# violetdenim/c3dgs

Hardware: AMD Instinct MI355X
Metric: raster views/sec fwd+bwd @1920x1080 (higher is better)
Workload: dtype f32; 1 GPU; BASELINE.json configs[2]: synth-v1 3M Gaussians, SH deg 3, indexed-camera rasterizer (QAT inner loop), mark_visible+fwd+bwd, 1 view/step/GPU; gaussians=3000000, width=1920, height=1080, sh_codebook=304096, gaussian_codebook=754096, parallelism=replicas x1

## Files before the change

c3dgs_amd/csrc/binning.hip:

```cpp
#include "common.hpp"
#include <rocprim/device/device_radix_sort.hpp>
#include <rocprim/iterator/counting_iterator.hpp>

namespace c3dgs {

size_t scan_temp_bytes(int P)
{
    size_t a = 0, b = 0;
    (void)rocprim::radix_sort_pairs(nullptr, b, (const uint32_t*)nullptr, (uint32_t*)nullptr, (const uint32_t*)nullptr,
                                    (uint32_t*)nullptr, (size_t)P, 0u, 32u);
    size_t m = a > b ? a : b;
    const size_t os = onesweep_depth_temp_bytes(P);
    if (os > m) m = os;
    return m < 256 ? 256 : m;
}

size_t sort_temp_bytes(int R, int end_bit, int key_bytes)
{
    size_t bytes = 0;
    if (key_bytes == 4)
        (void)rocprim::radix_sort_pairs(nullptr, bytes, (const uint32_t*)nullptr, (uint32_t*)nullptr,
                                        (const uint32_t*)nullptr, (uint32_t*)nullptr, (size_t)R, 0u, (unsigned)end_bit);
    else
        (void)rocprim::radix_sort_pairs(nullptr, bytes, (const uint16_t*)nullptr, (uint16_t*)nullptr,
                                        (const uint32_t*)nullptr, (uint32_t*)nullptr, (size_t)R, 0u, (unsigned)end_bit);
    const size_t os = onesweep_tile_temp_bytes(R, end_bit, key_bytes);
    if (os > bytes) bytes = os;
    const size_t reuse = align_up((size_t)(R > 0 ? R : 1));
    if (reuse > bytes) bytes = reuse;
    return bytes < 256 ? 256 : bytes;
}

__global__ void __launch_bounds__(256)
gather_u64_kernel(int n, const uint32_t* __restrict__ idx, const uint2* __restrict__ src, uint2* __restrict__ dst)
{
    const int i = blockIdx.x * 256 + threadIdx.x;
    if (i < n) dst[i] = src[idx[i]];
}

size_t depth_sort_clear_bytes(int P)
{
    return (onesweep_enabled() && (size_t)P < ((size_t)1 << 30)) ? onesweep_depth_clear_bytes(P) : 0;
}
size_t tile_sort_clear_bytes(int R, int end_bit, int key_bytes)
{
    return (onesweep_enabled() && (size_t)R < ((size_t)1 << 30)) ? onesweep_tile_clear_bytes(R, end_bit, key_bytes) : 0;
}

hipError_t run_depth_sort(void* temp, size_t temp_bytes, const uint32_t* kin, uint32_t* kout, const uint32_t* vin,
                          uint32_t* vout, int P, const uint2* rects, uint2* rects_sorted, hipStream_t s, bool ctrl_cleared,
                          bool rects_fit_bytes)
{
    if (onesweep_enabled() && (size_t)P < ((size_t)1 << 30))
        return onesweep_depth_sort(temp, temp_bytes, kin, kout, vin, vout, P, rects, rects_sorted, s, ctrl_cleared, rects_fit_bytes);
    hipError_t e = vin ? rocprim::radix_sort_pairs(temp, temp_bytes, kin, kout, vin, vout, (size_t)P, 0u, 32u, s)
                       : rocprim::radix_sort_pairs(temp, temp_bytes, kin, kout, rocprim::counting_iterator<uint32_t>(0u), vout,
                                                   (size_t)P, 0u, 32u, s);
    if (e != hipSuccess) return e;
    gather_u64_kernel<<<(P + 255) / 256, 256, 0, s>>>(P, vout, rects, rects_sorted);
    return hipGetLastError();
}

hipError_t run_tile_sort(void* temp, size_t temp_bytes, const void* kin, void* kout, int key_bytes, const uint32_t* vin,
                         uint32_t* vout, int R, int end_bit, hipStream_t s, bool ctrl_cleared)
{
    if (key_bytes == 4) {
        if (onesweep_enabled() && (size_t)R < ((size_t)1 << 30))
            return onesweep_tile_sort32(temp, temp_bytes, (const uint32_t*)kin, (uint32_t*)kout, vin, vout, R, end_bit, s, ctrl_cleared);
        return rocprim::radix_sort_pairs(temp, temp_bytes, (const uint32_t*)kin, (uint32_t*)kout, vin, vout, (size_t)R, 0u, (unsigned)end_bit, s);
    }
    if (onesweep_enabled() && (size_t)R < ((size_t)1 << 30))
        return onesweep_tile_sort(temp, temp_bytes, (const uint16_t*)kin, (uint16_t*)kout, vin, vout, R, end_bit, s, ctrl_cleared);
    return rocprim::radix_sort_pairs(temp, temp_bytes, (const uint16_t*)kin, (uint16_t*)kout, vin, vout, (size_t)R, 0u, (unsigned)end_bit, s);
}

}
```

c3dgs_amd/csrc/c_abi.hip:

```cpp
#include "common.hpp"
#include <cstdlib>
#include <cstring>
#include <mutex>
#include <vector>

namespace c3dgs {

static thread_local std::string g_last_error;
void set_error(const std::string& msg) { g_last_error = msg; }

enum Stage { ST_MARK_VISIBLE, ST_PREPROCESS, ST_DEPTH_SORT, ST_SCAN, ST_DUPLICATE, ST_SORT, ST_RANGES, ST_RENDER_FWD, ST_ZERO_PARTIALS,
             ST_RENDER_BWD, ST_BWD_PREPROCESS, ST_WDIST, ST_VQ_ACC, ST_VQ_APPLY, ST_LOSS_FWD, ST_LOSS_BWD,
             ST_QAT_OBSERVE, ST_QAT_CODEBOOKS, ST_QAT_VISIBLE, ST_QAT_POINTS, ST_QAT_POINTS_BWD, ST_QAT_CODEBOOKS_BWD, ST_ADAM, ST_COUNT };
static const char* kStageNames[ST_COUNT] = { "mark_visible", "preprocess", "depth_sort", "scan", "duplicate_with_keys", "sort",
                                             "identify_ranges", "render_forward", "zero_partials", "render_backward",
                                             "backward_preprocess", "weighted_distance", "vq_accumulate", "vq_apply", "l1_ssim_forward",
                                             "l1_ssim_backward", "qat_observe", "qat_codebooks", "qat_visible", "qat_points",
                                             "qat_points_backward", "qat_codebooks_backward", "adam_step" };
struct ProfRec { int stage; hipEvent_t a, b; };
static std::mutex g_prof_mu;
static bool g_prof_on = false;
static int g_prof_only = -1;
static std::vector<ProfRec> g_prof_recs;
static std::vector<hipEvent_t> g_prof_pool;

struct StageTimer {
    bool on; int stage; hipStream_t s; hipEvent_t a{}, b{};
    StageTimer(int stage_, hipStream_t s_) : on(g_prof_on && (g_prof_only < 0 || g_prof_only == stage_)), stage(stage_), s(s_)
    {
        if (!on) return;
        std::lock_guard<std::mutex> lk(g_prof_mu);
        auto get = [&](hipEvent_t& e) {
            if (!g_prof_pool.empty()) { e = g_prof_pool.back(); g_prof_pool.pop_back(); }
            else if (hipEventCreate(&e) != hipSuccess) on = false;
        };
        get(a); get(b);
        if (on) (void)hipEventRecord(a, s);
    }
    ~StageTimer()
    {
        if (!on) return;
        (void)hipEventRecord(b, s);
        std::lock_guard<std::mutex> lk(g_prof_mu);
        g_prof_recs.push_back({ stage, a, b });
    }
};

struct HostRead {
    uint32_t* pinned = nullptr;
    uint32_t* dev = nullptr;
    uint32_t seq = 0;
    hipEvent_t ev{};
    HostRead()
    {
        const char* e = std::getenv("C3DGS_HOST_READ_COPY");
        const bool want_map = !(e && e[0] == '1');
        if (want_map && hipHostMalloc((void**)&pinned, 64, hipHostMallocMapped | hipHostMallocPortable | hipHostMallocCoherent) == hipSuccess) {
            void* d = nullptr;
            if (hipHostGetDevicePointer(&d, pinned, 0) == hipSuccess) dev = (uint32_t*)d;
            std::memset(pinned, 0, 64);
        } else {
            (void)hipGetLastError();
            if (hipHostMalloc((void**)&pinned, 64, hipHostMallocDefault) != hipSuccess) { pinned = nullptr; return; }
        }
        if (hipEventCreateWithFlags(&ev, hipEventDisableTiming) != hipSuccess) { (void)hipHostFree(pinned); pinned = nullptr; dev = nullptr; }
    }
};
static HostRead& host_read()
{
    static thread_local HostRead h;
    return h;
}

static int validate(const c3dgs_raster_params* p, bool indexed, bool is_backward)
{
    if (!p) return fail(C3DGS_E_INVALID, "params is NULL");
    if (p->P < 0 || p->W <= 0 || p->H <= 0) return fail(C3DGS_E_INVALID, "P, W, H must be non-negative / positive");
    if (p->P == 0) return C3DGS_OK;
    if (!p->means3D) return fail(C3DGS_E_INVALID, "means3D must have dimensions (num_points, 3)");
    if (!p->background || !p->viewmatrix || !p->projmatrix || !p->campos)
        return fail(C3DGS_E_INVALID, "background, viewmatrix, projmatrix and campos are required");
    if (!is_backward && !p->opacities)
        return fail(C3DGS_E_INVALID, "opacities is required");
    if ((p->sh == nullptr) == (p->colors_precomp == nullptr))
        return fail(C3DGS_E_INVALID, "Please provide excatly one of either SHs or precomputed colors!");
    const bool has_sr = p->scales != nullptr && p->rotations != nullptr;
    if ((p->scales != nullptr) != (p->rotations != nullptr) || has_sr == (p->cov3D_precomp != nullptr))
        return fail(C3DGS_E_INVALID, "Please provide exactly one of either scale/rotation pair or precomputed 3D covariance!");
    if (p->sh) {
        if (p->D < 0 || p->D > 3) return fail(C3DGS_E_INVALID, "SH degree must be in [0,3]");
        if (p->M < (p->D + 1) * (p->D + 1)) return fail(C3DGS_E_INVALID, "sh has fewer coefficients than the active degree needs");
    }
    if (indexed) {
        if (p->sh && !p->sh_indices) return fail(C3DGS_E_INVALID, "indexed rasterizer: sh_indices is required with sh");
        if (has_sr && (!p->g_indices || !p->scale_factors))
            return fail(C3DGS_E_INVALID, "indexed rasterizer: g_indices and scale_factors are required with scales/rotations");
    } else if (p->sh_indices || p->g_indices || p->scale_factors) {
        return fail(C3DGS_E_INVALID, "non-indexed rasterizer: sh_indices / g_indices / scale_factors must be NULL");
    }
    if (tiles_x(p->W) > 65535 || tiles_y(p->H) > 65535) return fail(C3DGS_E_INVALID, "image too large for 16-bit tile coordinates");
    if ((unsigned long long)tiles_x(p->W) * tiles_x(p->W) * tiles_y(p->H) >= (1ull << 32))
        return fail(C3DGS_E_INVALID, "image too large: (tiles per row)^2 x (tile rows) must stay below 2^32");
    return C3DGS_OK;
}

static int forward_impl(const c3dgs_raster_params* pp, bool indexed, c3dgs_resize_fn geom_resize, void* geom_user,
                        c3dgs_resize_fn binning_resize, void* binning_user, c3dgs_resize_fn image_resize, void* image_user,
                        float* out_color, int32_t* radii, int32_t* num_rendered, void* stream_)
{
    if (int rc = validate(pp, indexed, false)) return rc;
    if (!out_color || !num_rendered) return fail(C3DGS_E_INVALID, "out_color and num_rendered are required");
    if (!geom_resize || !binning_resize || !image_resize) return fail(C3DGS_E_INVALID, "resize callbacks are required");
    c3dgs_raster_params p = *pp;
    if (!indexed) { p.sh_indices = nullptr; p.g_indices = nullptr; p.scale_factors = nullptr; }
    hipStream_t s = (hipStream_t)stream_;
    const int P = p.P, W = p.W, H = p.H;
    const int gx = tiles_x(W), gy = tiles_y(H), T = gx * gy;
    *num_rendered = 0;

    c3dgs_image_layout IL; image_layout(W, H, &IL);
    void* img_base = image_resize(image_user, IL.total_bytes);
    if (!img_base) return fail(C3DGS_E_ALLOC, "image buffer allocation failed");
    const ImgPtrs img = img_ptrs(img_base, W, H);

    if (P == 0) {
        C3DGS_HIP_TRY(hipMemsetAsync(out_color, 0, (size_t)3 * W * H * sizeof(float), s));
        C3DGS_HIP_TRY(hipMemsetAsync(img_base, 0, IL.total_bytes, s));
        return C3DGS_OK;
    }
    if (!radii) return fail(C3DGS_E_INVALID, "radii is required");

    c3dgs_geom_layout GL; geom_layout(P, &GL);
    void* geom_base = geom_resize(geom_user, GL.total_bytes + geom_gtab_bytes(p));
    if (!geom_base) return fail(C3DGS_E_ALLOC, "geometry buffer allocation failed");
    const GeomPtrs g = geom_ptrs(geom_base, P);

    uint32_t* sort_err = onesweep_error_word();
    if (!sort_err) return fail(C3DGS_E_HIP, "cannot resolve the sort error word");
    HostRead& hr = host_read();
    if (!hr.pinned) return fail(C3DGS_E_HIP, "pinned host buffer allocation failed");
    const uint32_t seq = hr.dev ? ++hr.seq : 0u;
    if (hr.dev && seq == 0u) hr.seq = 1u;
    const uint32_t want_seq = hr.dev ? hr.seq : 0u;
    const size_t dclear = depth_sort_clear_bytes(P) <= g.scan_temp_bytes ? depth_sort_clear_bytes(P) : 0;
    { StageTimer t_(ST_PREPROCESS, s);
      if (geom_gtab_bytes(p)) launch_pack_codebook(p, g.gtab, s);
      launch_preprocess(p, g, radii, img.ranges, sort_err, g.scan_temp, dclear / 16, hr.dev, want_seq, s); }
    C3DGS_STAGE("preprocess", p.debug, s);
    if (!hr.dev) {
        C3DGS_HIP_TRY(hipMemcpyAsync(hr.pinned, g.block_base + (P + 255) / 256, 2 * sizeof(uint32_t), hipMemcpyDeviceToHost, s));
        C3DGS_HIP_TRY(hipEventRecord(hr.ev, s));
    }
    { StageTimer t_(ST_DEPTH_SORT, s);
      C3DGS_HIP_TRY(run_depth_sort(g.scan_temp, g.scan_temp_bytes, g.depth_keys, g.depth_keys_sorted, nullptr, g.depth_order, P,
                                   reinterpret_cast<const uint2*>(g.rects), g.sorted_offsets, s, dclear != 0,
                                   gx <= 255 && gy <= 255)); }
    C3DGS_STAGE("depth_sort", p.debug, s);
    if (p.debug && onesweep_timed_out(s)) return fail(C3DGS_E_HIP, "depth sort: look-back timed out");
    { StageTimer t_(ST_SCAN, s); launch_depth_order_scan(P, g, s); }
    C3DGS_STAGE("scan", p.debug, s);
    if (hr.dev) {
        volatile uint32_t* pad = hr.pinned;
        bool seen = false;
        for (long spins = 0; !seen; spins++) {
            seen = __atomic_load_n(&pad[2], __ATOMIC_ACQUIRE) == want_seq;
            if (!seen && (spins & 0xffff) == 0xffff) {
                const hipError_t q = hipStreamQuery(s);
                if (q == hipErrorNotReady) continue;
                if (q != hipSuccess) return fail(C3DGS_E_HIP, std::string("num_rendered read: ") + hipGetErrorString(q));
                seen = __atomic_load_n(&pad[2], __ATOMIC_ACQUIRE) == want_seq;
                if (!seen) {
                    C3DGS_HIP_TRY(hipMemcpyAsync(hr.pinned, g.block_base + (P + 255) / 256, 2 * sizeof(uint32_t), hipMemcpyDeviceToHost, s));
                    C3DGS_HIP_TRY(hipStreamSynchronize(s));
                    seen = true;
                }
            }
        }
    } else {
        hipError_t q = hipErrorNotReady;
        for (long spins = 0; spins < 20000000L && (q = hipEventQuery(hr.ev)) == hipErrorNotReady; spins++) { }
        if (q == hipErrorNotReady) q = hipEventSynchronize(hr.ev);
        if (q != hipSuccess) return fail(C3DGS_E_HIP, std::string("num_rendered read: ") + hipGetErrorString(q));
    }
    const uint32_t R_u = hr.pinned[0];
    if (hr.pinned[1] != 0) {
        C3DGS_HIP_TRY(hipMemsetAsync(sort_err, 0, sizeof(uint32_t), s));
        return fail(C3DGS_E_HIP, "radix sort look-back timed out in an earlier rasterizer call on this device: that call's "
                                 "image is NaN and its gradients are invalid (flag cleared, this call was not run)");
    }
    if (R_u > 0x7fffffffu) return fail(C3DGS_E_INVALID, "num_rendered overflows int32");
    const int R = (int)R_u;
    *num_rendered = R;

    c3dgs_binning_layout BL; binning_layout(R, W, H, &BL);
    void* bin_base = binning_resize(binning_user, BL.total_bytes);
    if (!bin_base) return fail(C3DGS_E_ALLOC, "binning buffer allocation failed");
    const BinPtrs b = bin_ptrs(bin_base, R, W, H);

    if (R > 0) {
        const int end_bit = (int)higher_msb((uint32_t)T);
        size_t tclear = tile_sort_clear_bytes(R, end_bit, b.key_bytes);
        if (tclear > b.sort_temp_bytes) tclear = 0;
        { StageTimer t_(ST_DUPLICATE, s); launch_duplicate_with_keys(P, g, b, gx, sort_err, b.sort_temp, tclear / 16, s); }
        C3DGS_STAGE("duplicate_with_keys", p.debug, s);
        { StageTimer t_(ST_SORT, s);
          C3DGS_HIP_TRY(run_tile_sort(b.sort_temp, b.sort_temp_bytes, b.keys_unsorted, b.keys_sorted, b.key_bytes, b.values_unsorted,
                                      b.point_list, R, end_bit, s, tclear != 0)); }
        C3DGS_STAGE("sort", p.debug, s);
        if (p.debug && onesweep_timed_out(s)) return fail(C3DGS_E_HIP, "tile sort: look-back timed out");
        { StageTimer t_(ST_RANGES, s); launch_identify_ranges(R, b.keys_sorted, b.key_bytes, img.ranges, sort_err, s); }
        C3DGS_STAGE("identify_ranges", p.debug, s);
    }
    { StageTimer t_(ST_RENDER_FWD, s);
      launch_render_forward(W, H, img, b.point_list, g.splat, p.background, out_color, (uint8_t*)b.sort_temp, sort_err, s); }
    C3DGS_STAGE("render_forward", p.debug, s);
    return C3DGS_OK;
}

static int backward_impl(const c3dgs_raster_params* pp, bool indexed, const int32_t* radii, const void* geom_buffer,
                         const void* binning_buffer, const void* image_buffer, int32_t R, const float* dL_dout_color,
                         c3dgs_resize_fn ws_resize, void* ws_user, const c3dgs_raster_grads* grads, void* stream_)
{
    if (int rc = validate(pp, indexed, true)) return rc;
    if (!grads) return fail(C3DGS_E_INVALID, "grads is NULL");
    c3dgs_raster_params p = *pp;
    if (!indexed) { p.sh_indices = nullptr; p.g_indices = nullptr; p.scale_factors = nullptr; }
    hipStream_t s = (hipStream_t)stream_;
    const int P = p.P, W = p.W, H = p.H;

    void* cb_zero = nullptr;
    size_t cb_zero16 = 0;
    if (indexed) {
        const size_t n_sh = (grads->dL_dsh && p.sh) ? (size_t)p.SHS * p.M * 3 * sizeof(float) : 0;
        const size_t n_rot = (grads->dL_drotations && p.scales) ? (size_t)p.GS * 4 * sizeof(float) : 0;
        const size_t n_sc = (grads->dL_dscales && p.scales) ? (size_t)p.GS * 3 * sizeof(float) : 0;
        char* a_sh = (char*)grads->dL_dsh; char* a_rot = (char*)grads->dL_drotations; char* a_sc = (char*)grads->dL_dscales;
        if (n_sh && n_rot && n_sc && a_rot == a_sh + n_sh && a_sc == a_rot + n_rot) {
            const size_t n = n_sh + n_rot + n_sc;
            if (p.P > 0 && R >= 0 && ((uintptr_t)a_sh & 15u) == 0) {
                cb_zero = a_sh; cb_zero16 = n / 16;
                if (n % 16) C3DGS_HIP_TRY(hipMemsetAsync(a_sh + cb_zero16 * 16, 0, n % 16, s));
            } else {
                C3DGS_HIP_TRY(hipMemsetAsync(a_sh, 0, n, s));
            }
        } else {
            if (n_sh) C3DGS_HIP_TRY(hipMemsetAsync(a_sh, 0, n_sh, s));
            if (n_sc) C3DGS_HIP_TRY(hipMemsetAsync(a_sc, 0, n_sc, s));
            if (n_rot) C3DGS_HIP_TRY(hipMemsetAsync(a_rot, 0, n_rot, s));
        }
    }
    if (P == 0) return C3DGS_OK;
    if (!radii || !geom_buffer || !image_buffer || !dL_dout_color || (R > 0 && !binning_buffer))
        return fail(C3DGS_E_INVALID, "radii, forward buffers and dL_dout_color are required");
    if (!ws_resize) return fail(C3DGS_E_INVALID, "workspace callback is required");
    if (R < 0) return fail(C3DGS_E_INVALID, "R must be >= 0");

    const GeomPtrs g = geom_ptrs(const_cast<void*>(geom_buffer), P);
    const ImgPtrs img = img_ptrs(const_cast<void*>(image_buffer), W, H);
    const size_t ws_bytes = c3dgs_backward_workspace_bytes(P, R);
    float* partials = (float*)ws_resize(ws_user, ws_bytes);
    if (!partials) return fail(C3DGS_E_ALLOC, "backward workspace allocation failed");

    const size_t r1 = (size_t)(R > 0 ? R : 1), p256 = ((size_t)P + 1023) / 1024 * 1024;
    uint8_t* touched = (uint8_t*)partials + align_up(r1 * PARTIAL_FLOATS * sizeof(float));
    uint32_t* tile_order = img.tile_order;
    uint32_t* live_ids = (uint32_t*)(touched + align_up(r1)) + 65536;
    uint32_t* live_slots = live_ids + p256;
    uint32_t* live_count = live_slots + p256;
    { StageTimer t_(ST_ZERO_PARTIALS, s);
      launch_backward_prep(R > 0 ? W : 0, H, img, tile_order, touched, align_up(r1) / 16, R > 0 ? nullptr : cb_zero,
                           R > 0 ? 0 : cb_zero16, s); }
    if (R > 0) {
        const BinPtrs b = bin_ptrs(const_cast<void*>(binning_buffer), R, W, H);
        { StageTimer t_(ST_RENDER_BWD, s);
          launch_render_backward(W, H, img, b.point_list, g.splat, g.block_base, p.background, dL_dout_color, partials, touched,
                                 (const uint8_t*)b.sort_temp, tile_order, cb_zero, cb_zero16, s); }
        C3DGS_STAGE("render_backward", p.debug, s);
    }
    { StageTimer t_(ST_BWD_PREPROCESS, s);
      launch_backward_preprocess(p, radii, g, partials, touched, live_count, live_ids, live_slots, *grads, s); }
    C3DGS_STAGE("backward_preprocess", p.debug, s);
    return C3DGS_OK;
}

}

using namespace c3dgs;

extern "C" {

const char* c3dgs_last_error(void) { return g_last_error.c_str(); }

int c3dgs_profile_enable(int on)
{
    std::lock_guard<std::mutex> lk(g_prof_mu);
    g_prof_on = on != 0;
    return C3DGS_OK;
}

int c3dgs_profile_only(const char* stage_name)
{
    std::lock_guard<std::mutex> lk(g_prof_mu);
    g_prof_only = -1;
    if (!stage_name || !*stage_name) return C3DGS_OK;
    for (int i = 0; i < ST_COUNT; i++)
        if (std::strcmp(stage_name, kStageNames[i]) == 0) { g_prof_only = i; return C3DGS_OK; }
    return fail(C3DGS_E_INVALID, std::string("profile_only: unknown stage ") + stage_name);
}

int c3dgs_profile_read(c3dgs_stage_time* out, int capacity)
{
    std::vector<ProfRec> recs;
    {
        std::lock_guard<std::mutex> lk(g_prof_mu);
        recs.swap(g_prof_recs);
    }
    double total[ST_COUNT] = { 0 };
    long long count[ST_COUNT] = { 0 };
    for (auto& r : recs) {
        float ms = 0.f;
        if (hipEventSynchronize(r.b) == hipSuccess && hipEventElapsedTime(&ms, r.a, r.b) == hipSuccess) {
            total[r.stage] += (double)ms;
            count[r.stage]++;
        }
    }
    {
        std::lock_guard<std::mutex> lk(g_prof_mu);
        for (auto& r : recs) { g_prof_pool.push_back(r.a); g_prof_pool.push_back(r.b); }
    }
    int n = 0;
    for (int i = 0; i < ST_COUNT && n < capacity; i++) {
        if (!count[i]) continue;
        std::memset(&out[n], 0, sizeof(out[n]));
        std::strncpy(out[n].name, kStageNames[i], sizeof(out[n].name) - 1);
        out[n].total_ms = total[i];
        out[n].count = count[i];
        n++;
    }
    return n;
}
int c3dgs_abi_version(void) { return C3DGS_ABI_VERSION; }

int c3dgs_debug_sort_times(uint64_t* out )
{
    unsigned long long v[512];
    if (!out || os_read_times(v)) return fail(C3DGS_E_INVALID, "debug_sort_times: not a C3DGS_OS_TIMING build");
    for (int i = 0; i < 512; i++) out[i] = (uint64_t)v[i];
    return C3DGS_OK;
}

int c3dgs_debug_gather_probe(int32_t kind, int64_t n, void* table, const uint32_t* index, uint32_t* out, void* stream)
{
    if (n < 0 || !table || !out || (kind != 0 && !index)) return fail(C3DGS_E_INVALID, "debug_gather_probe: bad arguments");
    if (launch_gather_probe(kind, (size_t)n, table, index, out, (hipStream_t)stream)) return fail(C3DGS_E_INVALID, "debug_gather_probe: kind must be 0..3");
    return C3DGS_OK;
}

int c3dgs_debug_lane_counters(uint64_t* out, void* stream)
{
    if (!out) return fail(C3DGS_E_INVALID, "debug_lane_counters: NULL buffer");
    unsigned long long v[16];
    if (read_lane_counters(v, (hipStream_t)stream)) return fail(C3DGS_E_HIP, "debug_lane_counters: copy failed");
    for (int i = 0; i < 16; i++) out[i] = (uint64_t)v[i];
    return C3DGS_OK;
}

size_t c3dgs_debug_sort_temp_bytes(int32_t key_bytes, int64_t n, int32_t end_bit)
{
    if (n <= 0 || n > 0x3fffffff) return 256;
    return key_bytes == 2 ? onesweep_tile_temp_bytes((int)n, end_bit) : onesweep_depth_temp_bytes((int)n);
}

int c3dgs_debug_sort_pairs(int32_t key_bytes, int64_t n, int32_t end_bit, const void* keys_in, void* keys_out,
                           const uint32_t* values_in, uint32_t* values_out, void* temp, size_t temp_bytes, void* stream)
{
    if ((key_bytes != 2 && key_bytes != 4) || n < 0 || n > 0x3fffffff || end_bit < 1 || end_bit > 8 * key_bytes)
        return fail(C3DGS_E_INVALID, "debug_sort_pairs: bad arguments");
    if (key_bytes == 4 && end_bit != 32) return fail(C3DGS_E_INVALID, "debug_sort_pairs: 4-byte keys are sorted on all 32 bits");
    if (n == 0) return C3DGS_OK;
    if (!keys_in || !keys_out || !values_in || !values_out || !temp) return fail(C3DGS_E_INVALID, "debug_sort_pairs: NULL buffer");
    hipStream_t s = (hipStream_t)stream;
    if (key_bytes == 2)
        C3DGS_HIP_TRY(onesweep_tile_sort(temp, temp_bytes, (const uint16_t*)keys_in, (uint16_t*)keys_out, values_in, values_out, (int)n,
                                         end_bit, s));
    else
        C3DGS_HIP_TRY(onesweep_depth_sort(temp, temp_bytes, (const uint32_t*)keys_in, (uint32_t*)keys_out, values_in, values_out, (int)n,
                                          nullptr, nullptr, s));
    C3DGS_STAGE("debug_sort_pairs", 1, s);
    if (onesweep_timed_out(s)) return fail(C3DGS_E_HIP, "debug_sort_pairs: look-back timed out");
    return C3DGS_OK;
}

int c3dgs_get_geom_layout(int32_t P, c3dgs_geom_layout* out)
{
    if (!out || P < 0) return fail(C3DGS_E_INVALID, "bad arguments");
    geom_layout(P, out);
    return C3DGS_OK;
}
int c3dgs_get_binning_layout(int32_t R, int32_t W, int32_t H, c3dgs_binning_layout* out)
{
    if (!out || R < 0 || W <= 0 || H <= 0) return fail(C3DGS_E_INVALID, "bad arguments");
    binning_layout(R, W, H, out);
    return C3DGS_OK;
}
int c3dgs_get_image_layout(int32_t W, int32_t H, c3dgs_image_layout* out)
{
    if (!out || W <= 0 || H <= 0) return fail(C3DGS_E_INVALID, "bad arguments");
    image_layout(W, H, out);
    return C3DGS_OK;
}
size_t c3dgs_backward_workspace_bytes(int32_t P, int32_t R)
{
    const size_t r = (size_t)(R > 0 ? R : 1), p256 = ((size_t)(P > 0 ? P : 1) + 1023) / 1024 * 1024;
    return align_up(r * PARTIAL_FLOATS * sizeof(float)) + align_up(r) + 65536 * sizeof(uint32_t) +
           (2 * p256 + p256 / 256) * sizeof(uint32_t) + 256;
}

int c3dgs_mark_visible(int32_t P, const float* means3D, const float* viewmatrix, const float* projmatrix, uint8_t* present,
                       void* stream)
{
    (void)projmatrix;
    if (P < 0) return fail(C3DGS_E_INVALID, "P must be >= 0");
    if (P == 0) return C3DGS_OK;
    if (!means3D || !viewmatrix || !present) return fail(C3DGS_E_INVALID, "means3D, viewmatrix and present are required");
    { StageTimer t_(ST_MARK_VISIBLE, (hipStream_t)stream); launch_mark_visible(P, means3D, viewmatrix, present, (hipStream_t)stream); }
    C3DGS_STAGE("mark_visible", 0, (hipStream_t)stream);
    return C3DGS_OK;
}

int c3dgs_mark_visible_pose(int32_t P, const float* means3D, const float* extrinsic_vector, uint8_t* present, void* stream)
{
    if (P < 0) return fail(C3DGS_E_INVALID, "P must be >= 0");
    if (P == 0) return C3DGS_OK;
    if (!means3D || !extrinsic_vector || !present) return fail(C3DGS_E_INVALID, "means3D, extrinsic_vector and present are required");
    { StageTimer t_(ST_MARK_VISIBLE, (hipStream_t)stream); launch_mark_visible_pose(P, means3D, extrinsic_vector, present, (hipStream_t)stream); }
    C3DGS_STAGE("mark_visible", 0, (hipStream_t)stream);
    return C3DGS_OK;
}

int c3dgs_camera_from_pose(const float* extrinsic_vector, float inv_tan_half_fovx, float inv_tan_half_fovy, float* viewmatrix,
                           float* projmatrix, float* campos, void* stream)
{
    if (!extrinsic_vector || !viewmatrix || !projmatrix || !campos) return fail(C3DGS_E_INVALID, "camera_from_pose: NULL pointer");
    launch_camera_from_pose(extrinsic_vector, inv_tan_half_fovx, inv_tan_half_fovy, viewmatrix, projmatrix, campos, (hipStream_t)stream);
    C3DGS_STAGE("camera_from_pose", 0, (hipStream_t)stream);
    return C3DGS_OK;
}

int c3dgs_rasterize_gaussians(const c3dgs_raster_params* p, c3dgs_resize_fn geom_resize, void* geom_user,
                              c3dgs_resize_fn binning_resize, void* binning_user, c3dgs_resize_fn image_resize,
                              void* image_user, float* out_color, int32_t* radii, int32_t* num_rendered, void* stream)
{
    return forward_impl(p, false, geom_resize, geom_user, binning_resize, binning_user, image_resize, image_user, out_color,
                        radii, num_rendered, stream);
}

int c3dgs_rasterize_gaussians_indexed(const c3dgs_raster_params* p, c3dgs_resize_fn geom_resize, void* geom_user,
                                      c3dgs_resize_fn binning_resize, void* binning_user, c3dgs_resize_fn image_resize,
                                      void* image_user, float* out_color, int32_t* radii, int32_t* num_rendered, void* stream)
{
    return forward_impl(p, true, geom_resize, geom_user, binning_resize, binning_user, image_resize, image_user, out_color,
                        radii, num_rendered, stream);
}

int c3dgs_rasterize_gaussians_backward(const c3dgs_raster_params* p, const int32_t* radii, const void* geom_buffer,
                                       const void* binning_buffer, const void* image_buffer, int32_t R,
                                       const float* dL_dout_color, c3dgs_resize_fn workspace_resize, void* workspace_user,
                                       const c3dgs_raster_grads* grads, void* stream)
{
    return backward_impl(p, false, radii, geom_buffer, binning_buffer, image_buffer, R, dL_dout_color, workspace_resize,
                         workspace_user, grads, stream);
}

int c3dgs_rasterize_gaussians_backward_indexed(const c3dgs_raster_params* p, const int32_t* radii, const void* geom_buffer,
                                               const void* binning_buffer, const void* image_buffer, int32_t R,
                                               const float* dL_dout_color, c3dgs_resize_fn workspace_resize,
                                               void* workspace_user, const c3dgs_raster_grads* grads, void* stream)
{
    return backward_impl(p, true, radii, geom_buffer, binning_buffer, image_buffer, R, dL_dout_color, workspace_resize,
                         workspace_user, grads, stream);
}

int c3dgs_weighted_distance(int64_t N, int32_t C, int32_t K, const float* coefs, const int64_t* gather,
                            const float* codebook, float* out_dist, int64_t* out_idx, void* stream)
{
    if (N < 0 || C < 0 || K <= 0) return fail(C3DGS_E_INVALID, "coefs and codebook must have same number of channels");
    if (N == 0) return C3DGS_OK;
    if (!coefs || !codebook || !out_dist || !out_idx) return fail(C3DGS_E_INVALID, "ceofs and codebook must have dimension 2");
    {
        StageTimer t_(ST_WDIST, (hipStream_t)stream);
        if (launch_weighted_distance(N, C, K, coefs, gather, codebook, out_dist, out_idx, (hipStream_t)stream))
            return fail(C3DGS_E_INVALID, "unsupported channel count");
    }
    C3DGS_STAGE("weighted_distance", 0, (hipStream_t)stream);
    return C3DGS_OK;
}

size_t c3dgs_weighted_distance_ws_bytes(int64_t N, int32_t C, int32_t K) { return wd_ws_bytes(N, C, K); }

int c3dgs_weighted_distance_ws(int64_t N, int32_t C, int32_t K, const float* coefs, const int64_t* gather, const float* codebook,
                               float* out_dist, int64_t* out_idx, void* ws, size_t ws_bytes, void* stream)
{
    if (N < 0 || C < 0 || K <= 0) return fail(C3DGS_E_INVALID, "coefs and codebook must have same number of channels");
    if (N == 0) return C3DGS_OK;
    if (!coefs || !codebook || !out_dist || !out_idx) return fail(C3DGS_E_INVALID, "ceofs and codebook must have dimension 2");
    {
        StageTimer t_(ST_WDIST, (hipStream_t)stream);
        if (launch_weighted_distance(N, C, K, coefs, gather, codebook, out_dist, out_idx, (hipStream_t)stream, ws, ws ? ws_bytes : 0))
            return fail(C3DGS_E_INVALID, "unsupported channel count");
    }
    C3DGS_STAGE("weighted_distance", 0, (hipStream_t)stream);
    return C3DGS_OK;
}

int c3dgs_vq_accumulate(int64_t B, int32_t K, int32_t D, const float* x, const float* w, const int64_t* gather,
                        const int64_t* idx, const float* dist, float* S, double* dist_sum, void* stream)
{
    if (B < 0 || K <= 0 || D <= 0) return fail(C3DGS_E_INVALID, "bad sizes");
    if (B == 0) return C3DGS_OK;
    if (!x || !w || !idx || !S) return fail(C3DGS_E_INVALID, "x, w, idx and S are required");
    { StageTimer t_(ST_VQ_ACC, (hipStream_t)stream); launch_vq_accumulate(B, K, D, x, w, gather, idx, dist, S, dist_sum, (hipStream_t)stream); }
    C3DGS_STAGE("vq_accumulate", 0, (hipStream_t)stream);
    return C3DGS_OK;
}

int c3dgs_vq_sums(int64_t B, int32_t K, int32_t D, const float* x, const float* w, const int64_t* gather,
                  const float* codebook, float* dist, int64_t* idx, float* S, double* dist_sum, void* ws, size_t ws_bytes,
                  void* stream)
{
    if (B < 0 || K <= 0 || D <= 0) return fail(C3DGS_E_INVALID, "bad sizes");
    if (!S || !dist_sum) return fail(C3DGS_E_INVALID, "S and dist_sum are required");
    C3DGS_HIP_TRY(hipMemsetAsync(S, 0, (size_t)K * (D + 1) * sizeof(float), (hipStream_t)stream));
    C3DGS_HIP_TRY(hipMemsetAsync(dist_sum, 0, sizeof(double), (hipStream_t)stream));
    if (B == 0) return C3DGS_OK;
    if (!x || !w || !codebook || !dist || !idx) return fail(C3DGS_E_INVALID, "x, w, codebook, dist and idx are required");
    {
        StageTimer t_(ST_WDIST, (hipStream_t)stream);
        if (launch_weighted_distance(B, K, D, x, gather, codebook, dist, idx, (hipStream_t)stream, ws, ws ? ws_bytes : 0))
            return fail(C3DGS_E_INVALID, "unsupported channel count");
    }
    C3DGS_STAGE("weighted_distance", 0, (hipStream_t)stream);
    return c3dgs_vq_accumulate(B, K, D, x, w, gather, idx, dist, S, dist_sum, stream);
}

int c3dgs_vq_step_supported(int32_t K, int32_t D, const float* x, const float* codebook, const void* ws, size_t ws_bytes)
{
    return (K > 0 && D > 0 && wd_presplit_supported(K, D, x, codebook, ws, ws_bytes)) ? 1 : 0;
}

int c3dgs_vq_step_sums(int32_t step, int64_t B, int32_t K, int32_t D, const float* x, const float* w, const int64_t* gather,
                       const float* codebook, float* dist, int64_t* idx, float* S, double* dist_sum, void* ws, size_t ws_bytes,
                       void* stream)
{
    hipStream_t s = (hipStream_t)stream;
    if (step < 0 || B <= 0 || K <= 0 || D <= 0) return fail(C3DGS_E_INVALID, "vq_step_sums: bad sizes");
    if (!x || !w || !codebook || !dist || !idx || !S || !dist_sum) return fail(C3DGS_E_INVALID, "vq_step_sums: NULL argument");
    if (!wd_presplit_supported(K, D, x, codebook, ws, ws_bytes))
        return fail(C3DGS_E_INVALID, "vq_step_sums: shape / scratch not served by the fused step (see c3dgs_vq_step_supported)");
    if (step == 0) {
        C3DGS_HIP_TRY(hipMemsetAsync(S, 0, (size_t)K * (D + 1) * sizeof(float), s));
        C3DGS_HIP_TRY(hipMemsetAsync(dist_sum, 0, sizeof(double), s));
    }
    {
        StageTimer t_(ST_WDIST, s);
        if (launch_weighted_distance(B, K, D, x, gather, codebook, dist, idx, s, ws, ws_bytes, step == 0 ? -1 : (step & 1)))
            return fail(C3DGS_E_INVALID, "vq_step_sums: unsupported shape");
        if (step == 0) launch_vq_seed_words(K, D, ws, s);
    }
    C3DGS_STAGE("weighted_distance", 0, s);
    { StageTimer t_(ST_VQ_ACC, s);
      launch_vq_accumulate(B, K, D, x, w, gather, idx, dist, S, dist_sum, s, vq_next_absmax_word(K, D, ws, step & 1)); }
    C3DGS_STAGE("vq_accumulate", 0, s);
    return C3DGS_OK;
}

int c3dgs_vq_step_apply(int32_t step, int32_t K, int32_t D, float* S, float* codebook, float* entry_importance, float decay,
                        float alpha, float eps, int32_t scale_normalize, void* ws, size_t ws_bytes, void* stream)
{
    if (step < 0 || K <= 0 || D <= 0 || !S || !codebook || !entry_importance) return fail(C3DGS_E_INVALID, "vq_step_apply: bad arguments");
    { StageTimer t_(ST_VQ_APPLY, (hipStream_t)stream);
      if (launch_vq_apply_split(K, D, S, codebook, entry_importance, decay, alpha, eps, scale_normalize, ws, ws_bytes, step & 1, (hipStream_t)stream))
          return fail(C3DGS_E_INVALID, "vq_step_apply: shape / scratch not served by the fused step (see c3dgs_vq_step_supported)"); }
    C3DGS_STAGE("vq_apply", 0, (hipStream_t)stream);
    return C3DGS_OK;
}

int c3dgs_debug_wd_scores(int64_t N, int32_t C, int32_t K, const float* coefs, const float* codebook, float* scores, void* ws,
                          size_t ws_bytes, float* out_dist, int64_t* out_idx, void* stream)
{
    if (!coefs || !codebook || !scores || !out_dist || !out_idx) return fail(C3DGS_E_INVALID, "debug_wd_scores: bad arguments");
    if (launch_wd_debug_scores(N, C, K, coefs, codebook, scores, ws, ws_bytes, out_dist, out_idx, (hipStream_t)stream))
        return fail(C3DGS_E_INVALID, "debug_wd_scores: K = 48, 1 <= N <= 256, C >= 32 and scratch of c3dgs_weighted_distance_ws_bytes");
    return C3DGS_OK;
}

int c3dgs_vq_apply(int32_t K, int32_t D, const float* S, float* codebook, float* entry_importance, float decay,
                   float alpha, float eps, int32_t scale_normalize, void* stream)
{
    if (K <= 0 || D <= 0 || !S || !codebook || !entry_importance) return fail(C3DGS_E_INVALID, "bad arguments");
    { StageTimer t_(ST_VQ_APPLY, (hipStream_t)stream); launch_vq_apply(K, D, S, codebook, entry_importance, decay, alpha, eps, scale_normalize, (hipStream_t)stream); }
    C3DGS_STAGE("vq_apply", 0, (hipStream_t)stream);
    return C3DGS_OK;
}

size_t c3dgs_morton_workspace_bytes(int32_t P) { return morton_workspace_bytes(P); }

int c3dgs_morton_order(int32_t P, const float* xyz, int64_t* codes, int64_t* order, void* workspace, void* stream)
{
    if (P < 0) return fail(C3DGS_E_INVALID, "P must be >= 0");
    if (P == 0) return C3DGS_OK;
    if (!xyz || !codes || !order || !workspace) return fail(C3DGS_E_INVALID, "morton_order: bad arguments");
    if (run_morton_order(P, xyz, codes, order, workspace, (hipStream_t)stream)) return fail(C3DGS_E_HIP, "morton_order failed");
    C3DGS_STAGE("morton_order", 0, (hipStream_t)stream);
    return C3DGS_OK;
}

int c3dgs_abs_accumulate(int64_t n, const float* g, float* acc, void* stream)
{
    if (n < 0 || (n > 0 && (!g || !acc))) return fail(C3DGS_E_INVALID, "abs_accumulate: bad arguments");
    launch_abs_accumulate(n, g, acc, (hipStream_t)stream);
    C3DGS_STAGE("abs_accumulate", 0, (hipStream_t)stream);
    return C3DGS_OK;
}

int c3dgs_adam_step(int32_t n_tensors, const c3dgs_adam_tensor* tensors, double beta1, double beta2, double eps, void* stream)
{
    if (n_tensors < 0 || n_tensors > C3DGS_ADAM_MAX_TENSORS) return fail(C3DGS_E_INVALID, "adam_step: between 0 and 16 tensors per call");
    if (n_tensors == 0) return C3DGS_OK;
    if (!tensors) return fail(C3DGS_E_INVALID, "adam_step: tensors is NULL");
    for (int k = 0; k < n_tensors; k++)
        if (tensors[k].n > 0 && (!tensors[k].param || !tensors[k].grad || !tensors[k].exp_avg || !tensors[k].exp_avg_sq))
            return fail(C3DGS_E_INVALID, "adam_step: NULL tensor pointer");
    { StageTimer t_(ST_ADAM, (hipStream_t)stream); launch_adam(n_tensors, tensors, beta1, beta2, eps, (hipStream_t)stream); }
    C3DGS_STAGE("adam_step", 0, (hipStream_t)stream);
    return C3DGS_OK;
}

int c3dgs_extract_rot_scale(int32_t n, const float* cov6, float* rot, float* scale, void* stream)
{
    if (n < 0) return fail(C3DGS_E_INVALID, "extract_rot_scale: n must be >= 0");
    if (n == 0) return C3DGS_OK;
    if (!cov6 || !rot || !scale || (reinterpret_cast<uintptr_t>(rot) & 15)) return fail(C3DGS_E_INVALID, "extract_rot_scale: bad arguments");
    launch_extract_rot_scale(n, cov6, rot, scale, (hipStream_t)stream);
    C3DGS_STAGE("extract_rot_scale", 0, (hipStream_t)stream);
    return C3DGS_OK;
}

int c3dgs_l1_ssim_forward(int32_t C, int32_t H, int32_t W, const float* img, const float* gt, float* dmaps, double* sums,
                          void* stream)
{
    if (C <= 0 || H <= 0 || W <= 0 || !img || !gt || !sums) return fail(C3DGS_E_INVALID, "l1_ssim_forward: bad arguments");
    hipStream_t s = (hipStream_t)stream;
    C3DGS_HIP_TRY(hipMemsetAsync(sums, 0, 128 * sizeof(double), s));
    const size_t n = (size_t)C * H * W;
    {
        StageTimer t_(ST_LOSS_FWD, s);
        launch_l1_ssim_forward(C, H, W, img, gt, dmaps, dmaps ? dmaps + n : nullptr, dmaps ? dmaps + 2 * n : nullptr, sums, s);
    }
    C3DGS_STAGE("l1_ssim_forward", 0, s);
    return C3DGS_OK;
}

int c3dgs_l1_ssim_value(const double* sums, double l1_scale, double ssim_scale, double constant, float* out, void* stream)
{
    if (!sums || !out) return fail(C3DGS_E_INVALID, "l1_ssim_value: bad arguments");
    launch_l1_ssim_value(sums, l1_scale, ssim_scale, constant, out, (hipStream_t)stream);
    C3DGS_STAGE("l1_ssim_value", 0, (hipStream_t)stream);
    return C3DGS_OK;
}

int c3dgs_l1_ssim_backward(int32_t C, int32_t H, int32_t W, const float* img, const float* gt, const float* dmaps,
                           const float* grad_loss, float l1_coeff, float ssim_coeff, float* dL_dimg, void* stream)
{
    if (C <= 0 || H <= 0 || W <= 0 || !img || !gt || !dmaps || !grad_loss || !dL_dimg)
        return fail(C3DGS_E_INVALID, "l1_ssim_backward: bad arguments");
    hipStream_t s = (hipStream_t)stream;
    const size_t n = (size_t)C * H * W;
    {
        StageTimer t_(ST_LOSS_BWD, s);
        launch_l1_ssim_backward(C, H, W, img, gt, dmaps, dmaps + n, dmaps + 2 * n, grad_loss, l1_coeff, ssim_coeff, dL_dimg, s);
    }
    C3DGS_STAGE("l1_ssim_backward", 0, s);
    return C3DGS_OK;
}

size_t c3dgs_image_metrics_ws_bytes(int32_t N, int32_t C, int32_t H, int32_t W) { return image_metrics_ws_bytes(N, C, H, W); }

int c3dgs_image_metrics(int32_t N, int32_t C, int32_t H, int32_t W, const float* img, const float* gt, void* ws, size_t ws_bytes,
                        double* out, void* stream)
{
    if (N <= 0 || C <= 0 || H <= 0 || W <= 0) return fail(C3DGS_E_INVALID, "image_metrics: N, C, H and W must be positive");
    if (image_metrics_workgroups(N, C, H, W) > IMAGE_METRICS_MAX_WORKGROUPS)
        return fail(C3DGS_E_INVALID, "image_metrics: size overflow (N * C * H * W too large for one call; split the batch)");
    if (!img || !gt || !ws || !out) return fail(C3DGS_E_INVALID, "image_metrics: img, gt, ws and out are required");
    if (reinterpret_cast<uintptr_t>(ws) & 7) return fail(C3DGS_E_INVALID, "image_metrics: ws must be 8-byte aligned");
    const size_t need = image_metrics_ws_bytes(N, C, H, W);
    if (ws_bytes < need)
        return fail(C3DGS_E_INVALID, "image_metrics: ws too small (" + std::to_string(ws_bytes) + " bytes, need " +
                                         std::to_string(need) + ")");
    launch_image_metrics(N, C, H, W, img, gt, (double*)ws, out, (hipStream_t)stream);
    C3DGS_STAGE("image_metrics", 0, (hipStream_t)stream);
    return C3DGS_OK;
}

static int qat_validate(const c3dgs_qat_params* q, const char* who)
{
    if (!q) return fail(C3DGS_E_INVALID, std::string(who) + ": params is NULL");
    if (q->P < 0 || q->GS < 0 || q->SHS < 0 || q->M < 1) return fail(C3DGS_E_INVALID, std::string(who) + ": bad sizes");
    if (!q->state) return fail(C3DGS_E_INVALID, std::string(who) + ": state is required");
    if (q->features_dc && q->M > 1 && !q->features_rest)
        return fail(C3DGS_E_INVALID, std::string(who) + ": features_rest is required with features_dc when M > 1");
    if (reinterpret_cast<uintptr_t>(q->rotation) & 15) return fail(C3DGS_E_INVALID, std::string(who) + ": rotation must be 16-byte aligned");
    return C3DGS_OK;
}
static bool misaligned16(const void* p) { return (reinterpret_cast<uintptr_t>(p) & 15) != 0; }

size_t c3dgs_qat_workspace_bytes(void) { return qat_workspace_bytes(); }
size_t c3dgs_qat_scan_bytes(int32_t P) { return qat_scan_bytes(P); }

int c3dgs_qat_observe(const c3dgs_qat_params* q, void* workspace, void* stream)
{
    if (int rc = qat_validate(q, "qat_observe")) return rc;
    if (!workspace) return fail(C3DGS_E_INVALID, "qat_observe: workspace is required");
    { StageTimer t_(ST_QAT_OBSERVE, (hipStream_t)stream); launch_qat_observe(*q, workspace, (hipStream_t)stream); }
    C3DGS_STAGE("qat_observe", 0, (hipStream_t)stream);
    return C3DGS_OK;
}

int c3dgs_qat_codebooks(const c3dgs_qat_params* q, float* scales_n, float* rotations, float* shs, void* stream)
{
    if (int rc = qat_validate(q, "qat_codebooks")) return rc;
    if (misaligned16(rotations) || misaligned16(shs)) return fail(C3DGS_E_INVALID, "qat_codebooks: outputs must be 16-byte aligned");
    { StageTimer t_(ST_QAT_CODEBOOKS, (hipStream_t)stream); launch_qat_codebooks(*q, scales_n, rotations, shs, (hipStream_t)stream); }
    C3DGS_STAGE("qat_codebooks", 0, (hipStream_t)stream);
    return C3DGS_OK;
}

int c3dgs_qat_codebooks_backward(const c3dgs_qat_params* q, const float* dL_dscales_n, const float* dL_drotations,
                                 const float* dL_dshs, float* dL_dscaling, float* dL_drotation, float* dL_dfeatures_dc,
                                 float* dL_dfeatures_rest, void* stream)
{
    if (int rc = qat_validate(q, "qat_codebooks_backward")) return rc;
    if (misaligned16(dL_drotations) || misaligned16(dL_drotation) || misaligned16(dL_dshs))
        return fail(C3DGS_E_INVALID, "qat_codebooks_backward: rotation / sh gradients must be 16-byte aligned");
    if (dL_dshs && q->features_dc && (!dL_dfeatures_dc || (q->M > 1 && !dL_dfeatures_rest)))
        return fail(C3DGS_E_INVALID, "qat_codebooks_backward: dL_dfeatures_dc / dL_dfeatures_rest are required with dL_dshs");
    {
        StageTimer t_(ST_QAT_CODEBOOKS_BWD, (hipStream_t)stream);
        launch_qat_codebooks_backward(*q, dL_dscales_n, dL_drotations, dL_dshs, dL_dscaling, dL_drotation, dL_dfeatures_dc,
                                      dL_dfeatures_rest, (hipStream_t)stream);
    }
    C3DGS_STAGE("qat_codebooks_backward", 0, (hipStream_t)stream);
    return C3DGS_OK;
}

int c3dgs_qat_visible(const c3dgs_qat_params* q, const float* viewmatrix, uint8_t* visible, int32_t* rank, int32_t* count,
                      void* scan_workspace, void* stream)
{
    if (int rc = qat_validate(q, "qat_visible")) return rc;
    if (!count) return fail(C3DGS_E_INVALID, "qat_visible: count is required");
    hipStream_t s = (hipStream_t)stream;
    if (q->P == 0) { C3DGS_HIP_TRY(hipMemsetAsync(count, 0, sizeof(int32_t), s)); return C3DGS_OK; }
    if (!q->xyz || !viewmatrix || !visible || !rank || !scan_workspace) return fail(C3DGS_E_INVALID, "qat_visible: bad arguments");
    { StageTimer t_(ST_QAT_VISIBLE, s); C3DGS_HIP_TRY(run_qat_visible(*q, viewmatrix, visible, rank, count, scan_workspace, s)); }
    C3DGS_STAGE("qat_visible", 0, s);
    return C3DGS_OK;
}

int c3dgs_qat_points(const c3dgs_qat_params* q, const uint8_t* visible, const int32_t* rank, const int64_t* sh_indices,
                     const int64_t* g_indices, float* means3D, float* opacities, float* scale_factors, int64_t* sh_indices_out,
                     int64_t* g_indices_out, void* stream)
{
    if (int rc = qat_validate(q, "qat_points")) return rc;
    if ((visible == nullptr) != (rank == nullptr)) return fail(C3DGS_E_INVALID, "qat_points: visible and rank go together");
    {
        StageTimer t_(ST_QAT_POINTS, (hipStream_t)stream);
        launch_qat_points(*q, visible, rank, sh_indices, g_indices, means3D, opacities, scale_factors, sh_indices_out,
                          g_indices_out, (hipStream_t)stream);
    }
    C3DGS_STAGE("qat_points", 0, (hipStream_t)stream);
    return C3DGS_OK;
}

int c3dgs_qat_points_backward(const c3dgs_qat_params* q, const uint8_t* visible, const int32_t* rank, const float* dL_dmeans3D,
                              const float* dL_dmeans2D, const float* dL_dopacities, const float* dL_dscale_factors,
                              float* dL_dxyz, float* dL_dscreenspace, float* dL_dopacity, float* dL_dscaling_factor, void* stream)
{
    if (int rc = qat_validate(q, "qat_points_backward")) return rc;
    if ((visible == nullptr) != (rank == nullptr)) return fail(C3DGS_E_INVALID, "qat_points_backward: visible and rank go together");
    if ((dL_dopacity && dL_dopacities && !q->opacity) || (dL_dscaling_factor && dL_dscale_factors && !q->scaling_factor))
        return fail(C3DGS_E_INVALID, "qat_points_backward: the raw opacity / scaling_factor are needed to recompute the masks");
    {
        StageTimer t_(ST_QAT_POINTS_BWD, (hipStream_t)stream);
        launch_qat_points_backward(*q, visible, rank, dL_dmeans3D, dL_dmeans2D, dL_dopacities, dL_dscale_factors, dL_dxyz,
                                   dL_dscreenspace, dL_dopacity, dL_dscaling_factor, (hipStream_t)stream);
    }
    C3DGS_STAGE("qat_points_backward", 0, (hipStream_t)stream);
    return C3DGS_OK;
}

int c3dgs_qat_quantize(const c3dgs_qat_params* q, int32_t scaling_is_exp, int8_t* opacity, int8_t* scaling, int8_t* scaling_factor,
                       int8_t* rotation, int8_t* features_dc, int8_t* features_rest, void* stream)
{
    if (int rc = qat_validate(q, "qat_quantize")) return rc;
    if (rotation && (reinterpret_cast<uintptr_t>(rotation) & 3)) return fail(C3DGS_E_INVALID, "qat_quantize: rotation output must be 4-byte aligned");
    launch_qat_quantize(*q, scaling_is_exp, opacity, scaling, scaling_factor, rotation, features_dc, features_rest, (hipStream_t)stream);
    C3DGS_STAGE("qat_quantize", 0, (hipStream_t)stream);
    return C3DGS_OK;
}

int c3dgs_fake_quantize(int64_t n, const float* x, c3dgs_fq_state* state, int32_t observe, int32_t enabled,
                        float averaging_constant, float* out, void* workspace, void* stream)
{
    if (n < 0) return fail(C3DGS_E_INVALID, "fake_quantize: n must be >= 0");
    if (n == 0) return C3DGS_OK;
    if (!x || !state || !out || (observe && !workspace)) return fail(C3DGS_E_INVALID, "fake_quantize: bad arguments");
    launch_fake_quantize(n, x, state, observe, enabled, averaging_constant, out, workspace, (hipStream_t)stream);
    C3DGS_STAGE("fake_quantize", 0, (hipStream_t)stream);
    return C3DGS_OK;
}

int c3dgs_fake_quantize_backward(int64_t n, const float* x, const c3dgs_fq_state* state, int32_t enabled, const float* g,
                                 float* dx, void* stream)
{
    if (n < 0) return fail(C3DGS_E_INVALID, "fake_quantize_backward: n must be >= 0");
    if (n == 0) return C3DGS_OK;
    if (!x || !state || !g || !dx) return fail(C3DGS_E_INVALID, "fake_quantize_backward: bad arguments");
    launch_fake_quantize_backward(n, x, state, enabled, g, dx, (hipStream_t)stream);
    C3DGS_STAGE("fake_quantize_backward", 0, (hipStream_t)stream);
    return C3DGS_OK;
}

}
```

c3dgs_amd/csrc/common.hpp:

```cpp
#pragma once
#include <hip/hip_runtime.h>
#include <cstdint>
#include <cstddef>
#include <cstdio>
#include <cstring>
#include <string>

#include "../../include/c3dgs_hip.h"

namespace c3dgs {

constexpr int TILE = 16;
constexpr int TILE_PIX = 256;
constexpr int SPLAT_F4 = 3;
constexpr int PARTIAL_FLOATS = 9;

void set_error(const std::string& msg);
inline int fail(int code, const std::string& msg) { set_error(msg); return code; }

#define C3DGS_HIP_TRY(expr)                                                                         \
    do {                                                                                            \
        hipError_t e__ = (expr);                                                                    \
        if (e__ != hipSuccess)                                                                      \
            return ::c3dgs::fail(C3DGS_E_HIP, std::string(#expr) + ": " + hipGetErrorString(e__));  \
    } while (0)

#define C3DGS_STAGE(name, debug, stream)                                                            \
    do {                                                                                            \
        hipError_t e__ = hipGetLastError();                                                         \
        if (e__ == hipSuccess && (debug)) e__ = hipStreamSynchronize(stream);                       \
        if (e__ != hipSuccess)                                                                      \
            return ::c3dgs::fail(C3DGS_E_HIP, std::string("stage ") + name + ": " + hipGetErrorString(e__)); \
    } while (0)

inline size_t align_up(size_t v, size_t a = 256) { return (v + a - 1) / a * a; }

size_t scan_temp_bytes(int P);
size_t sort_temp_bytes(int R, int end_bit, int key_bytes = 2);

inline int tiles_x(int W) { return (W + TILE - 1) / TILE; }
inline int tiles_y(int H) { return (H + TILE - 1) / TILE; }

inline uint32_t higher_msb(uint32_t n)
{
    uint32_t msb = sizeof(n) * 4, step = msb;
    while (step > 1) {
        step /= 2;
        if (n >> msb) msb += step; else msb -= step;
    }
    if (n >> msb) msb++;
    return msb;
}

inline void geom_layout(int P, c3dgs_geom_layout* L)
{
    size_t o = 0, p = (size_t)(P > 0 ? P : 1);
    L->splat = o;             o = align_up(o + p * SPLAT_F4 * 16);
    L->depth_keys = o;        o = align_up(o + p * 4);
    L->depth_keys_sorted = o; o = align_up(o + p * 4);
    L->depth_order = o;       o = align_up(o + p * 4);
    L->sorted_offsets = o;    o = align_up(o + p * 8);
    L->inst_offset = o;       o = align_up(o + p * 4);
    L->rects = o;             o = align_up(o + p * 8);
    L->clamped = o;           o = align_up(o + p);
    L->block_base = o;        o = align_up(o + ((p + 255) / 256 + 2) * 4);
    L->depth_base = o;        o = align_up(o + ((p + 255) / 256 + 1) * 4);
    L->scan_temp = o;         L->scan_temp_bytes = scan_temp_bytes((int)p);
    o = align_up(o + L->scan_temp_bytes);
    L->total_bytes = o;
}

inline size_t geom_gtab_bytes(const c3dgs_raster_params& p) { return (p.g_indices && p.scales) ? align_up((size_t)(p.GS > 0 ? p.GS : 1) * 32) : 0; }

inline int tile_key_bytes(int W, int H) { return (long long)tiles_x(W) * tiles_y(H) > 65536 ? 4 : 2; }

inline void binning_layout(int R, int W, int H, c3dgs_binning_layout* L)
{
    size_t o = 0, r = (size_t)(R > 0 ? R : 1);
    int end_bit = (int)higher_msb((uint32_t)(tiles_x(W) * tiles_y(H)));
    const size_t kb = (size_t)tile_key_bytes(W, H);
    L->keys_unsorted = o;   o = align_up(o + r * kb);
    L->values_unsorted = o; o = align_up(o + r * 4);
    L->keys_sorted = o;     o = align_up(o + r * kb);
    L->point_list = o;      o = align_up(o + r * 4);
    L->sort_temp = o;       L->sort_temp_bytes = sort_temp_bytes((int)r, end_bit, (int)kb);
    o = align_up(o + L->sort_temp_bytes);
    L->total_bytes = o;
}

inline void image_layout(int W, int H, c3dgs_image_layout* L)
{
    size_t o = 0, n = (size_t)W * H, t = (size_t)tiles_x(W) * tiles_y(H);
    L->final_T = o;   o = align_up(o + n * 4);
    L->n_contrib = o; o = align_up(o + n * 4);
    L->ranges = o;    o = align_up(o + t * 8);
    L->tile_used = o; o = align_up(o + t * 4);
    L->tile_order = o; o = align_up(o + t * 4);
    L->total_bytes = o;
}

struct GeomPtrs {
    float4* splat; uint32_t* depth_keys; uint32_t* depth_keys_sorted;
    uint32_t* depth_order; uint2* sorted_offsets; uint32_t* inst_offset; uint16_t* rects;
    uint8_t* clamped; uint32_t* block_base; uint32_t* depth_base; void* scan_temp; size_t scan_temp_bytes;
    float4* gtab;
};
struct BinPtrs {
    void* keys_unsorted; uint32_t* values_unsorted; void* keys_sorted; uint32_t* point_list;
    void* sort_temp; size_t sort_temp_bytes; int key_bytes;
};
struct ImgPtrs { float* final_T; uint32_t* n_contrib; uint2* ranges; uint32_t* tile_used; uint32_t* tile_order; };

inline GeomPtrs geom_ptrs(void* base, int P)
{
    c3dgs_geom_layout L; geom_layout(P, &L);
    char* b = (char*)base;
    return { (float4*)(b + L.splat), (uint32_t*)(b + L.depth_keys), (uint32_t*)(b + L.depth_keys_sorted), (uint32_t*)(b + L.depth_order),
             (uint2*)(b + L.sorted_offsets), (uint32_t*)(b + L.inst_offset), (uint16_t*)(b + L.rects),
             (uint8_t*)(b + L.clamped), (uint32_t*)(b + L.block_base), (uint32_t*)(b + L.depth_base), (void*)(b + L.scan_temp),
             L.scan_temp_bytes, (float4*)(b + L.total_bytes) };
}
inline BinPtrs bin_ptrs(void* base, int R, int W, int H)
{
    c3dgs_binning_layout L; binning_layout(R, W, H, &L);
    char* b = (char*)base;
    return { (void*)(b + L.keys_unsorted), (uint32_t*)(b + L.values_unsorted), (void*)(b + L.keys_sorted),
             (uint32_t*)(b + L.point_list), (void*)(b + L.sort_temp), L.sort_temp_bytes, tile_key_bytes(W, H) };
}
inline ImgPtrs img_ptrs(void* base, int W, int H)
{
    c3dgs_image_layout L; image_layout(W, H, &L);
    char* b = (char*)base;
    return { (float*)(b + L.final_T), (uint32_t*)(b + L.n_contrib), (uint2*)(b + L.ranges), (uint32_t*)(b + L.tile_used),
             (uint32_t*)(b + L.tile_order) };
}

void launch_camera_from_pose(const float* pose, float inv_tan_x, float inv_tan_y, float* view, float* proj, float* campos, hipStream_t s);
void launch_mark_visible(int P, const float* means3D, const float* view, uint8_t* present, hipStream_t s);
void launch_mark_visible_pose(int P, const float* means3D, const float* pose7, uint8_t* present, hipStream_t s);
void launch_pack_codebook(const c3dgs_raster_params& p, float4* gtab, hipStream_t s);
void launch_preprocess(const c3dgs_raster_params& p, const GeomPtrs& g, int32_t* radii, uint2* ranges, const uint32_t* sort_err,
                       void* zero_span, size_t zero_n16, uint32_t* host_out, uint32_t host_seq, hipStream_t s);
void launch_depth_order_scan(int P, const GeomPtrs& g, hipStream_t s);
void launch_duplicate_with_keys(int P, const GeomPtrs& g, const BinPtrs& b, int grid_x, const uint32_t* sort_err,
                                void* zero_span, size_t zero_n16, hipStream_t s);
void launch_identify_ranges(int R, const void* keys_sorted, int key_bytes, uint2* ranges, const uint32_t* sort_err, hipStream_t s);
hipError_t run_depth_sort(void* temp, size_t temp_bytes, const uint32_t* kin, uint32_t* kout, const uint32_t* vin,
                          uint32_t* vout, int P, const uint2* rects, uint2* rects_sorted, hipStream_t s, bool ctrl_cleared = false,
                          bool rects_fit_bytes = false);
hipError_t run_tile_sort(void* temp, size_t temp_bytes, const void* kin, void* kout, int key_bytes, const uint32_t* vin,
                         uint32_t* vout, int R, int end_bit, hipStream_t s, bool ctrl_cleared = false);
size_t depth_sort_clear_bytes(int P);
size_t tile_sort_clear_bytes(int R, int end_bit, int key_bytes);
bool onesweep_enabled();
int onesweep_timed_out(hipStream_t s);
uint32_t* onesweep_error_word();
size_t onesweep_depth_temp_bytes(int P);
size_t onesweep_tile_temp_bytes(int R, int end_bit, int key_bytes = 2);
size_t onesweep_depth_clear_bytes(int P);
size_t onesweep_tile_clear_bytes(int R, int end_bit, int key_bytes);
hipError_t onesweep_depth_sort(void* temp, size_t temp_bytes, const uint32_t* kin, uint32_t* kout, const uint32_t* vin, uint32_t* vout,
                               int P, const uint2* gather_src, uint2* gather_dst, hipStream_t s, bool ctrl_cleared = false,
                               bool rects_fit_bytes = false);
hipError_t onesweep_tile_sort32(void* temp, size_t temp_bytes, const uint32_t* kin, uint32_t* kout, const uint32_t* vin, uint32_t* vout,
                                int R, int end_bit, hipStream_t s, bool ctrl_cleared = false);
hipError_t onesweep_tile_sort(void* temp, size_t temp_bytes, const uint16_t* kin, uint16_t* kout, const uint32_t* vin, uint32_t* vout,
                              int R, int end_bit, hipStream_t s, bool ctrl_cleared = false);
int os_read_times(unsigned long long* out512);
int read_lane_counters(unsigned long long* out16, hipStream_t s);
void launch_render_forward(int W, int H, const ImgPtrs& img, const uint32_t* point_list, const float4* splat,
                           const float* bg, float* out_color, uint8_t* qmask, const uint32_t* sort_err, hipStream_t s);
void launch_backward_prep(int W, int H, const ImgPtrs& img, uint32_t* tile_order, void* zero_a, size_t n16_a, void* zero_b,
                          size_t n16_b, hipStream_t s);
void launch_render_backward(int W, int H, const ImgPtrs& img, const uint32_t* point_list, const float4* splat,
                            const uint32_t* block_base, const float* bg, const float* dL_dpix, float* partials,
                            uint8_t* touched, const uint8_t* qmask, const uint32_t* tile_order, void* zero_span, size_t zero_n16,
                            hipStream_t s);
void launch_backward_preprocess(const c3dgs_raster_params& p, const int32_t* radii, const GeomPtrs& g,
                                float* partials, const uint8_t* touched, uint32_t* live_count, uint32_t* live_ids,
                                uint32_t* live_slots, const c3dgs_raster_grads& gr, hipStream_t s);
int launch_weighted_distance(int64_t N, int C, int K, const float* coefs, const int64_t* gather, const float* codebook,
                             float* out_dist, int64_t* out_idx, hipStream_t s, void* ws = nullptr, size_t ws_bytes = 0, int presplit = -1);
bool wd_presplit_supported(int C, int K, const float* coefs, const float* codebook, const void* ws, size_t ws_bytes);
int launch_vq_apply_split(int K, int D, float* S, float* codebook, float* entry_importance, float decay, float alpha, float eps,
                          int scale_normalize, void* ws, size_t ws_bytes, int parity, hipStream_t s);
void launch_vq_seed_words(int K, int D, void* ws, hipStream_t s);
uint32_t* vq_next_absmax_word(int K, int D, void* ws, int parity);
size_t wd_ws_bytes(int64_t N, int C, int K);
int launch_wd_debug_scores(int64_t N, int C, int K, const float* coefs, const float* codebook, float* scores, void* ws, size_t ws_bytes,
                           float* out_dist, int64_t* out_idx, hipStream_t s);
void launch_vq_accumulate(int64_t B, int K, int D, const float* x, const float* w, const int64_t* gather,
                          const int64_t* idx, const float* dist, float* S, double* dist_sum, hipStream_t s, uint32_t* clear_word = nullptr);
void launch_vq_apply(int K, int D, const float* S, float* codebook, float* entry_importance, float decay, float alpha,
                     float eps, int scale_normalize, hipStream_t s);

int launch_gather_probe(int kind, size_t n, void* table, const uint32_t* index, uint32_t* out, hipStream_t s);
size_t morton_workspace_bytes(int P);
int run_morton_order(int P, const float* xyz, int64_t* codes_out, int64_t* order_out, void* workspace, hipStream_t s);
void launch_extract_rot_scale(int n, const float* cov6, float* rot, float* scale, hipStream_t s);
void launch_adam(int n_tensors, const c3dgs_adam_tensor* tensors, double beta1, double beta2, double eps, hipStream_t s);
void launch_abs_accumulate(int64_t n, const float* g, float* acc, hipStream_t s);
void launch_l1_ssim_value(const double* sums, double l1_scale, double ssim_scale, double constant, float* out, hipStream_t s);
void launch_l1_ssim_forward(int C, int H, int W, const float* img, const float* gt, float* Dmu, float* Ds1, float* Ds12,
                            double* sums, hipStream_t s);
void launch_l1_ssim_backward(int C, int H, int W, const float* img, const float* gt, const float* Dmu, const float* Ds1,
                             const float* Ds12, const float* grad_loss, float l1_coeff, float ssim_coeff, float* dL_dimg,
                             hipStream_t s);
constexpr int64_t IMAGE_METRICS_MAX_WORKGROUPS = (int64_t(1) << 24) - 1;
int64_t image_metrics_workgroups(int N, int C, int H, int W);
size_t image_metrics_ws_bytes(int N, int C, int H, int W);
void launch_image_metrics(int N, int C, int H, int W, const float* img, const float* gt, double* partials, double* out,
                          hipStream_t s);

size_t qat_workspace_bytes();
size_t qat_scan_bytes(int P);
void launch_qat_observe(const c3dgs_qat_params& q, void* workspace, hipStream_t s);
void launch_qat_codebooks(const c3dgs_qat_params& q, float* scales_n, float* rotations, float* shs, hipStream_t s);
void launch_qat_codebooks_backward(const c3dgs_qat_params& q, const float* g_scales, const float* g_rot, const float* g_shs,
                                   float* d_scaling, float* d_rotation, float* d_dc, float* d_rest, hipStream_t s);
hipError_t run_qat_visible(const c3dgs_qat_params& q, const float* view, uint8_t* visible, int32_t* rank, int32_t* count,
                           void* scan_ws, hipStream_t s);
void launch_qat_points(const c3dgs_qat_params& q, const uint8_t* visible, const int32_t* rank, const int64_t* sh_idx,
                       const int64_t* g_idx, float* means3D, float* opac, float* sfac, int64_t* sh_out, int64_t* g_out,
                       hipStream_t s);
void launch_qat_points_backward(const c3dgs_qat_params& q, const uint8_t* visible, const int32_t* rank, const float* g_m3,
                                const float* g_m2, const float* g_op, const float* g_sf, float* d_xyz, float* d_screen,
                                float* d_op, float* d_sf, hipStream_t s);
void launch_qat_quantize(const c3dgs_qat_params& q, int scaling_exp, int8_t* opacity, int8_t* scaling, int8_t* scaling_factor,
                         int8_t* rotation, int8_t* features_dc, int8_t* features_rest, hipStream_t s);
void launch_fake_quantize(long long n, const float* x, c3dgs_fq_state* state, int observe, int enabled, float c, float* out,
                          void* workspace, hipStream_t s);
void launch_fake_quantize_backward(long long n, const float* x, const c3dgs_fq_state* state, int enabled, const float* g,
                                   float* dx, hipStream_t s);

}
```

c3dgs_amd/csrc/preprocess.hip:

```cpp
#include "common.hpp"
#include "gsmath.hpp"

namespace c3dgs {

template <bool POSE>
__global__ void __launch_bounds__(256)
mark_visible_kernel(int P, const float* __restrict__ means3D, const float* __restrict__ view_or_pose, uint8_t* __restrict__ present, int vec)
{
    const int j = blockIdx.x * 256 + threadIdx.x;
    const int i0 = 4 * j;
    if (i0 >= P) return;
    float vm[16];
    const float* view = view_or_pose;
    if (POSE) {
        const float x = view_or_pose[0], y = view_or_pose[1], z = view_or_pose[2], w = view_or_pose[3], tz = view_or_pose[6];
        const float d2 = y * y + z * z + x * x;
#pragma unroll
        for (int q = 0; q < 16; q++) vm[q] = 0.f;
        vm[2] = 2.0f * (x * z - w * y); vm[6] = 2.0f * (y * z + w * x); vm[10] = 1.0f + 2.0f * (z * z - d2); vm[14] = tz;
        view = vm;
    }
    if (vec && i0 + 4 <= P) {
        const float4* src = reinterpret_cast<const float4*>(means3D) + 3 * (size_t)j;
        const float4 a = src[0], b = src[1], c = src[2];
        const f3 p0 = { a.x, a.y, a.z }, p1 = { a.w, b.x, b.y }, p2 = { b.z, b.w, c.x }, p3 = { c.y, c.z, c.w };
        const uint32_t v0 = !(xform4x3(p0, view).z <= 0.01f), v1 = !(xform4x3(p1, view).z <= 0.01f);
        const uint32_t v2 = !(xform4x3(p2, view).z <= 0.01f), v3 = !(xform4x3(p3, view).z <= 0.01f);
        reinterpret_cast<uint32_t*>(present)[j] = v0 | (v1 << 8) | (v2 << 16) | (v3 << 24);
        return;
    }
    for (int i = i0; i < min(i0 + 4, P); i++) {
        f3 p = { means3D[3 * (size_t)i], means3D[3 * (size_t)i + 1], means3D[3 * (size_t)i + 2] };
        f3 pv = xform4x3(p, view);
        present[i] = !(pv.z <= 0.01f) ? 1 : 0;
    }
}

__global__ void __launch_bounds__(256)
pack_codebook_kernel(int GS, const float* __restrict__ scales, const float* __restrict__ rotations, float4* __restrict__ gtab)
{
    const int g = blockIdx.x * 256 + threadIdx.x;
    if (g >= GS) return;
    gtab[2 * (size_t)g] = *reinterpret_cast<const float4*>(rotations + 4 * (size_t)g);
    gtab[2 * (size_t)g + 1] = make_float4(scales[3 * (size_t)g], scales[3 * (size_t)g + 1], scales[3 * (size_t)g + 2], 0.f);
}

void launch_pack_codebook(const c3dgs_raster_params& p, float4* gtab, hipStream_t s)
{
    if (p.GS <= 0) return;
    pack_codebook_kernel<<<(p.GS + 255) / 256, 256, 0, s>>>(p.GS, p.scales, p.rotations, gtab);
}

void launch_mark_visible(int P, const float* means3D, const float* view, uint8_t* present, hipStream_t s)
{
    if (P <= 0) return;
    const int vec = ((reinterpret_cast<uintptr_t>(means3D) & 15u) == 0 && (reinterpret_cast<uintptr_t>(present) & 3u) == 0) ? 1 : 0;
    mark_visible_kernel<false><<<((P + 3) / 4 + 255) / 256, 256, 0, s>>>(P, means3D, view, present, vec);
}

void launch_mark_visible_pose(int P, const float* means3D, const float* pose, uint8_t* present, hipStream_t s)
{
    if (P <= 0) return;
    const int vec = ((reinterpret_cast<uintptr_t>(means3D) & 15u) == 0 && (reinterpret_cast<uintptr_t>(present) & 3u) == 0) ? 1 : 0;
    mark_visible_kernel<true><<<((P + 3) / 4 + 255) / 256, 256, 0, s>>>(P, means3D, pose, present, vec);
}

__global__ void camera_from_pose_kernel(const float* __restrict__ pose, float inv_tan_x, float inv_tan_y, float pa, float pb,
                                        float* __restrict__ view, float* __restrict__ proj, float* __restrict__ campos)
{
    if (threadIdx.x != 0 || blockIdx.x != 0) return;
    const float x = pose[0], y = pose[1], z = pose[2], w = pose[3], tx = pose[4], ty = pose[5], tz = pose[6];
    const float d2 = y * y + z * z + x * x;
    float M[4][4];
    M[0][0] = 1.0f + 2.0f * (x * x - d2); M[0][1] = 2.0f * (x * y - w * z);        M[0][2] = 2.0f * (x * z + w * y);        M[0][3] = tx;
    M[1][0] = 2.0f * (x * y + w * z);        M[1][1] = 1.0f + 2.0f * (y * y - d2); M[1][2] = 2.0f * (y * z - w * x);        M[1][3] = ty;
    M[2][0] = 2.0f * (x * z - w * y);        M[2][1] = 2.0f * (y * z + w * x);        M[2][2] = 1.0f + 2.0f * (z * z - d2); M[2][3] = tz;
    M[3][0] = 0.f; M[3][1] = 0.f; M[3][2] = 0.f; M[3][3] = 1.f;
#pragma unroll
    for (int i = 0; i < 4; i++) {
#pragma unroll
        for (int j = 0; j < 4; j++) view[i * 4 + j] = M[j][i];
        proj[i * 4 + 0] = M[0][i] * inv_tan_x;
        proj[i * 4 + 1] = M[1][i] * inv_tan_y;
        proj[i * 4 + 2] = M[2][i] * pa + M[3][i] * pb;
        proj[i * 4 + 3] = M[2][i];
    }
    const double a = M[0][0], b = M[0][1], c = M[0][2], d = M[1][0], e = M[1][1], f = M[1][2], g = M[2][0], h = M[2][1], k = M[2][2];
    const double A = e * k - f * h, B = -(d * k - f * g), C = d * h - e * g;
    const double det = a * A + b * B + c * C;
    const double inv[3][3] = { { A / det, -(b * k - c * h) / det, (b * f - c * e) / det },
                               { B / det, (a * k - c * g) / det, -(a * f - c * d) / det },
                               { C / det, -(a * h - b * g) / det, (a * e - b * d) / det } };
#pragma unroll
    for (int r = 0; r < 3; r++) campos[r] = (float)-(inv[r][0] * (double)tx + inv[r][1] * (double)ty + inv[r][2] * (double)tz);
}

void launch_camera_from_pose(const float* pose, float inv_tan_x, float inv_tan_y, float* view, float* proj, float* campos, hipStream_t s)
{
    const float pa = (float)(1.0 * 100.0 / (100.0 - 0.01)), pb = (float)(-(100.0 * 0.01) / (100.0 - 0.01));
    camera_from_pose_kernel<<<1, 64, 0, s>>>(pose, inv_tan_x, inv_tan_y, pa, pb, view, proj, campos);
}

template <int DEG>
__device__ __forceinline__ void sh_to_rgb(const float* c, float x, float y, float z, float out[3])
{
#pragma unroll
    for (int ch = 0; ch < 3; ch++) {
        float res = SH_C0 * c[0 * 3 + ch];
        if (DEG > 0) {
            res = res - SH_C1 * y * c[1 * 3 + ch] + SH_C1 * z * c[2 * 3 + ch] - SH_C1 * x * c[3 * 3 + ch];
            if (DEG > 1) {
                float xx = x * x, yy = y * y, zz = z * z;
                float xy = x * y, yz = y * z, xz = x * z;
                res = res + SH_C2_0 * xy * c[4 * 3 + ch] + SH_C2_1 * yz * c[5 * 3 + ch] +
                      SH_C2_2 * (2.0f * zz - xx - yy) * c[6 * 3 + ch] + SH_C2_3 * xz * c[7 * 3 + ch] +
                      SH_C2_4 * (xx - yy) * c[8 * 3 + ch];
                if (DEG > 2) {
                    res = res + SH_C3_0 * y * (3.0f * xx - yy) * c[9 * 3 + ch] + SH_C3_1 * xy * z * c[10 * 3 + ch] +
                          SH_C3_2 * y * (4.0f * zz - xx - yy) * c[11 * 3 + ch] +
                          SH_C3_3 * z * (2.0f * zz - 3.0f * xx - 3.0f * yy) * c[12 * 3 + ch] +
                          SH_C3_4 * x * (4.0f * zz - xx - yy) * c[13 * 3 + ch] + SH_C3_5 * z * (xx - yy) * c[14 * 3 + ch] +
                          SH_C3_6 * x * (xx - 3.0f * yy) * c[15 * 3 + ch];
                }
            }
        }
        out[ch] = res + 0.5f;
    }
}

struct PreArgs {
    int P, M, W, H, gx, gy;
    const float* means3D; const float* sh; const float* colors_precomp; const float* opacities;
    const float* scales; const float* scale_factors; const float* rotations; const float* cov3D_precomp;
    const int64_t* sh_indices; const int64_t* g_indices;
    const float* view; const float* proj; const float* campos;
    float tan_fovx, tan_fovy, focal_x, focal_y, scale_modifier;
    int prefiltered, clamp_color;
    int32_t* radii; float4* splat; uint16_t* rects; uint8_t* clamped;
    uint32_t* depth_keys;
    uint32_t* inst_offset; uint32_t* block_total;
    uint2* ranges; int T;
    const float4* gtab;
    uint4* zero_span; size_t zero_n16;
};

template <int DEG>
__global__ void __launch_bounds__(256) preprocess_kernel(const PreArgs a)
{
    __shared__ uint32_t s_wsum[4];
    const int t = threadIdx.x, lane = t & 63, wave = t >> 6;
    const int i = blockIdx.x * 256 + t;
    const bool in_range = i < a.P;
    for (int q = i; q < a.T; q += gridDim.x * 256) a.ranges[q] = make_uint2(0u, 0u);
    if (a.zero_n16) {
        const size_t per = (a.zero_n16 + gridDim.x - 1) / gridDim.x, z0 = (size_t)blockIdx.x * per, z1 = min(z0 + per, a.zero_n16);
        for (size_t q = z0 + t; q < z1; q += 256) a.zero_span[q] = make_uint4(0u, 0u, 0u, 0u);
    }

    int32_t out_radius = 0;
    uint32_t out_tiles = 0;
    uint32_t out_key = 0xffffffffu;
    bool alive = false;
    float4 rec0 = make_float4(0, 0, 0, 0), rec1 = rec0;
    float rgb2 = 0.f;
    uint32_t rect_lo = 0, rect_hi = 0;
    if (in_range) do {
        const f3 p = { a.means3D[3 * (size_t)i], a.means3D[3 * (size_t)i + 1], a.means3D[3 * (size_t)i + 2] };
        const f3 p_view = xform4x3(p, a.view);
        if (!a.prefiltered && p_view.z <= 0.01f) break;

        const float4 p_hom = xform4x4(p, a.proj);
        const float p_w = 1.0f / (p_hom.w + 0.0000001f);
        const float projx = p_hom.x * p_w, projy = p_hom.y * p_w;

        float cov3D[6];
        if (a.cov3D_precomp) {
#pragma unroll
            for (int q = 0; q < 6; q++) cov3D[q] = a.cov3D_precomp[6 * (size_t)i + q];
        } else if (a.g_indices) {
            const size_t g = (size_t)a.g_indices[i];
            const float4 rot = a.gtab[2 * g], sc = a.gtab[2 * g + 1];
            cov3d_from_scale_rot(sc.x, sc.y, sc.z, a.scale_factors[i] * a.scale_modifier, rot, cov3D);
        } else {
            const float4 rot = *reinterpret_cast<const float4*>(a.rotations + 4 * (size_t)i);
            cov3d_from_scale_rot(a.scales[3 * (size_t)i], a.scales[3 * (size_t)i + 1], a.scales[3 * (size_t)i + 2],
                                 a.scale_modifier, rot, cov3D);
        }
        const Cov2D cv = cov2d(p, a.focal_x, a.focal_y, a.tan_fovx, a.tan_fovy, cov3D, a.view);

        const float det = (cv.a * cv.c - cv.b * cv.b);
        if (det == 0.0f) break;
        const float det_inv = 1.f / det;
        const float conic_a = cv.c * det_inv, conic_b = -cv.b * det_inv, conic_c = cv.a * det_inv;

        const float mid = 0.5f * (cv.a + cv.c);
        const float lambda1 = mid + sqrtf(fmaxf(0.1f, mid * mid - det));
        const float lambda2 = mid - sqrtf(fmaxf(0.1f, mid * mid - det));
        const float my_radius = ceilf(3.f * sqrtf(fmaxf(lambda1, lambda2)));
        const float pix = ndc2pix(projx, a.W), piy = ndc2pix(projy, a.H);
        int x0, y0, x1, y1;
        get_rect(pix, piy, (int)my_radius, a.gx, a.gy, x0, y0, x1, y1);
        if ((x1 - x0) * (y1 - y0) == 0) break;

        float rgb[3];
        uint8_t clamp_bits = 0;
        if (a.colors_precomp) {
            rgb[0] = a.colors_precomp[3 * (size_t)i];
            rgb[1] = a.colors_precomp[3 * (size_t)i + 1];
            rgb[2] = a.colors_precomp[3 * (size_t)i + 2];
        } else {
            const size_t row = a.sh_indices ? (size_t)a.sh_indices[i] : (size_t)i;
            const float* shp = a.sh + row * (size_t)a.M * 3;
            constexpr int NC = (DEG + 1) * (DEG + 1) * 3;
            float c[NC];
            if ((a.M * 3) % 4 == 0 && NC % 4 == 0) {
#pragma unroll
                for (int q = 0; q < NC / 4; q++) {
                    const float4 v = reinterpret_cast<const float4*>(shp)[q];
                    c[4 * q] = v.x; c[4 * q + 1] = v.y; c[4 * q + 2] = v.z; c[4 * q + 3] = v.w;
                }
            } else {
#pragma unroll
                for (int q = 0; q < NC; q++) c[q] = shp[q];
            }
            f3 dir = { p.x - a.campos[0], p.y - a.campos[1], p.z - a.campos[2] };
            const float len = sqrtf(dir.x * dir.x + dir.y * dir.y + dir.z * dir.z);
            dir.x = dir.x / len; dir.y = dir.y / len; dir.z = dir.z / len;
            sh_to_rgb<DEG>(c, dir.x, dir.y, dir.z, rgb);
            if (a.clamp_color) {
#pragma unroll
                for (int ch = 0; ch < 3; ch++) {
                    if (rgb[ch] < 0) clamp_bits |= (uint8_t)(1u << ch);
                    rgb[ch] = fmaxf(rgb[ch], 0.0f);
                }
            }
        }

        alive = true;
        out_radius = (int32_t)my_radius;
        out_tiles = (uint32_t)((y1 - y0) * (x1 - x0));
        out_key = __float_as_uint(p_view.z);
        a.clamped[i] = clamp_bits;
        uint16_t* rc = a.rects + 4 * (size_t)i;
        rc[0] = (uint16_t)x0; rc[1] = (uint16_t)y0; rc[2] = (uint16_t)x1; rc[3] = (uint16_t)y1;
        rec0 = make_float4(pix, piy, conic_a, conic_b);
        rec1 = make_float4(conic_c, a.opacities[i], rgb[0], rgb[1]);
        rgb2 = rgb[2];
        rect_lo = (uint32_t)x0 | ((uint32_t)y0 << 16);
        rect_hi = (uint32_t)x1 | ((uint32_t)y1 << 16);
    } while (false);

    uint32_t incl = out_tiles;
#pragma unroll
    for (int o = 1; o < 64; o <<= 1) { const uint32_t v = __shfl_up(incl, o); if (lane >= o) incl += v; }
    if (lane == 63) s_wsum[wave] = incl;
    __syncthreads();
    uint32_t woff = 0;
    for (int w = 0; w < wave; w++) woff += s_wsum[w];
    const uint32_t my_incl = woff + incl;
    if (t == 255) a.block_total[blockIdx.x] = my_incl;
    if (!in_range) return;
    if (!alive) *reinterpret_cast<uint2*>(a.rects + 4 * (size_t)i) = make_uint2(0u, 0u);
    if (alive) {
        float4* rec = a.splat + 3 * (size_t)i;
        rec[0] = rec0;
        rec[1] = rec1;
        rec[2] = make_float4(rgb2, __uint_as_float(my_incl - out_tiles), __uint_as_float(rect_lo), __uint_as_float(rect_hi));
    }
    a.inst_offset[i] = my_incl;
    a.radii[i] = out_radius;
    a.depth_keys[i] = out_key;
}

__global__ void __launch_bounds__(1024) scan_blocks_kernel(int nb, uint32_t* __restrict__ base, const uint32_t* __restrict__ sort_err,
                                                           uint32_t* __restrict__ host_out, uint32_t host_seq)
{
    __shared__ uint32_t s_w[2][16];
    const int t = threadIdx.x, lane = t & 63, wave = t >> 6;
    uint32_t carry = 0;
    int buf = 0;
    for (int c0 = 0; c0 < nb; c0 += 16384, buf ^= 1) {
        const int i0 = c0 + t * 16;
        uint32_t v[16];
#pragma unroll
        for (int q = 0; q < 4; q++) {
            uint4 x = make_uint4(0u, 0u, 0u, 0u);
            if (i0 + 4 * q + 3 < nb) x = reinterpret_cast<const uint4*>(base + i0)[q];
            else {
                if (i0 + 4 * q < nb) x.x = base[i0 + 4 * q];
                if (i0 + 4 * q + 1 < nb) x.y = base[i0 + 4 * q + 1];
                if (i0 + 4 * q + 2 < nb) x.z = base[i0 + 4 * q + 2];
            }
            v[4 * q] = x.x; v[4 * q + 1] = x.y; v[4 * q + 2] = x.z; v[4 * q + 3] = x.w;
        }
        uint32_t mine = 0;
#pragma unroll
        for (int q = 0; q < 16; q++) mine += v[q];
        uint32_t incl = mine;
#pragma unroll
        for (int o = 1; o < 64; o <<= 1) { const uint32_t u = __shfl_up(incl, o); if (lane >= o) incl += u; }
        if (lane == 63) s_w[buf][wave] = incl;
        __syncthreads();
        uint32_t off = carry, all = 0;
#pragma unroll
        for (int w = 0; w < 16; w++) { const uint32_t x = s_w[buf][w]; if (w < wave) off += x; all += x; }
        uint32_t run = off + incl - mine;
#pragma unroll
        for (int q = 0; q < 16; q++) { const uint32_t x = v[q]; v[q] = run; run += x; }
#pragma unroll
        for (int q = 0; q < 4; q++) {
            if (i0 + 4 * q + 3 < nb) reinterpret_cast<uint4*>(base + i0)[q] = make_uint4(v[4 * q], v[4 * q + 1], v[4 * q + 2], v[4 * q + 3]);
            else {
                if (i0 + 4 * q < nb) base[i0 + 4 * q] = v[4 * q];
                if (i0 + 4 * q + 1 < nb) base[i0 + 4 * q + 1] = v[4 * q + 1];
                if (i0 + 4 * q + 2 < nb) base[i0 + 4 * q + 2] = v[4 * q + 2];
            }
        }
        carry += all;
    }
    __syncthreads();
    if (t == 0) {
        base[nb] = carry;
        const uint32_t err = sort_err ? *sort_err : 0u;
        if (sort_err) base[nb + 1] = err;
        if (host_out) {
            __hip_atomic_store(host_out, carry, __ATOMIC_RELAXED, __HIP_MEMORY_SCOPE_SYSTEM);
            __hip_atomic_store(host_out + 1, err, __ATOMIC_RELAXED, __HIP_MEMORY_SCOPE_SYSTEM);
            __hip_atomic_store(host_out + 2, host_seq, __ATOMIC_RELEASE, __HIP_MEMORY_SCOPE_SYSTEM);
        }
    }
}

void launch_preprocess(const c3dgs_raster_params& p, const GeomPtrs& g, int32_t* radii, uint2* ranges, const uint32_t* sort_err,
                       void* zero_span, size_t zero_n16, uint32_t* host_out, uint32_t host_seq, hipStream_t s)
{
    if (p.P <= 0) return;
    PreArgs a;
    a.P = p.P; a.M = p.M; a.W = p.W; a.H = p.H; a.gx = tiles_x(p.W); a.gy = tiles_y(p.H);
    a.means3D = p.means3D; a.sh = p.sh; a.colors_precomp = p.colors_precomp; a.opacities = p.opacities;
    a.scales = p.scales; a.scale_factors = p.scale_factors; a.rotations = p.rotations; a.cov3D_precomp = p.cov3D_precomp;
    a.sh_indices = p.sh_indices; a.g_indices = p.g_indices;
    a.view = p.viewmatrix; a.proj = p.projmatrix; a.campos = p.campos;
    a.tan_fovx = p.tan_fovx; a.tan_fovy = p.tan_fovy;
    a.focal_y = p.H / (2.0f * p.tan_fovy);
    a.focal_x = p.W / (2.0f * p.tan_fovx);
    a.scale_modifier = p.scale_modifier; a.prefiltered = p.prefiltered; a.clamp_color = p.clamp_color;
    a.radii = radii; a.splat = g.splat; a.rects = g.rects;
    a.clamped = g.clamped; a.depth_keys = g.depth_keys;
    a.inst_offset = g.inst_offset;
    a.block_total = g.block_base;
    a.ranges = ranges; a.T = a.gx * a.gy;
    a.gtab = g.gtab;
    a.zero_span = (uint4*)zero_span; a.zero_n16 = zero_span ? zero_n16 : 0;
    const dim3 grid((p.P + 255) / 256), block(256);
    const int deg = p.colors_precomp ? 0 : p.D;
    switch (deg) {
        case 0: preprocess_kernel<0><<<grid, block, 0, s>>>(a); break;
        case 1: preprocess_kernel<1><<<grid, block, 0, s>>>(a); break;
        case 2: preprocess_kernel<2><<<grid, block, 0, s>>>(a); break;
        default: preprocess_kernel<3><<<grid, block, 0, s>>>(a); break;
    }
    scan_blocks_kernel<<<1, 1024, 0, s>>>((int)grid.x, g.block_base, sort_err, host_out, host_seq);
}

__device__ __forceinline__ uint32_t rect_tiles(const uint2 rc)
{
    return (uint32_t)(((int)(rc.y & 0xffff) - (int)(rc.x & 0xffff)) * ((int)(rc.y >> 16) - (int)(rc.x >> 16)));
}

__global__ void __launch_bounds__(256)
block_totals_kernel(int n, const uint2* __restrict__ rects_sorted, uint32_t* __restrict__ totals)
{
    __shared__ uint32_t s_w[4];
    const int i = blockIdx.x * 256 + threadIdx.x;
    uint32_t x = i < n ? rect_tiles(rects_sorted[i]) : 0u;
#pragma unroll
    for (int o = 32; o > 0; o >>= 1) x += __shfl_xor(x, o);
    if ((threadIdx.x & 63) == 0) s_w[threadIdx.x >> 6] = x;
    __syncthreads();
    if (threadIdx.x == 0) totals[blockIdx.x] = (s_w[0] + s_w[1]) + (s_w[2] + s_w[3]);
}

template <class K>
__global__ void __launch_bounds__(256)
duplicate_with_keys_kernel(int P, const uint32_t* __restrict__ order, const uint2* __restrict__ rects_sorted,
                           const uint32_t* __restrict__ depth_base, K* __restrict__ keys, uint32_t* __restrict__ values,
                           int grid_x, const uint32_t* __restrict__ sort_err, uint4* __restrict__ zero_span, size_t zero_n16)
{
    if (zero_n16) {
        const size_t per = (zero_n16 + gridDim.x - 1) / gridDim.x, z0 = (size_t)blockIdx.x * per, z1 = min(z0 + per, zero_n16);
        for (size_t q = z0 + threadIdx.x; q < z1; q += 256) zero_span[q] = make_uint4(0u, 0u, 0u, 0u);
    }
    if (*sort_err) return;
    __shared__ uint32_t s_end[256];
    __shared__ uint32_t s_id[256];
    __shared__ uint2 s_rect[256];
    __shared__ uint32_t s_inv[256];
    __shared__ uint32_t s_wsum[4];
    const int t = threadIdx.x, lane = t & 63, wave = t >> 6;
    const int k0 = blockIdx.x * 256, k = k0 + t;
    const uint32_t out_begin = depth_base[blockIdx.x];
    uint32_t incl = 0;
    if (k < P) {
        const uint2 rc = rects_sorted[k];
        incl = rect_tiles(rc);
        s_id[t] = order[k];
        s_rect[t] = rc;
        const uint32_t w = (rc.y & 0xffff) - (rc.x & 0xffff);
        s_inv[t] = w > 1 ? 0xffffffffu / w + 1u : 0u;
    }
#pragma unroll
    for (int o = 1; o < 64; o <<= 1) { const uint32_t v = __shfl_up(incl, o); if (lane >= o) incl += v; }
    if (lane == 63) s_wsum[wave] = incl;
    __syncthreads();
    uint32_t woff = out_begin;
    for (int w = 0; w < wave; w++) woff += s_wsum[w];
    s_end[t] = woff + incl;
    __syncthreads();
    const int nk = min(256, P - k0);
    const uint32_t out_end = s_end[nk - 1];
    constexpr int CH = 1024;
    __shared__ uint16_t s_head[CH];
    __shared__ uint32_t s_wmax[4];
    const uint32_t my_tiles = k < P ? rect_tiles(s_rect[t]) : 0u;
    const uint32_t my_begin = s_end[t] - my_tiles;
    uint32_t carry = 0;
    for (uint32_t c0 = out_begin & ~3u; c0 < out_end; c0 += CH) {
        reinterpret_cast<uint2*>(s_head)[t] = make_uint2(0u, 0u);
        __syncthreads();
        if (my_tiles && my_begin >= c0 && my_begin < c0 + CH) s_head[my_begin - c0] = (uint16_t)(t + 1);
        __syncthreads();
        const uint2 hv = reinterpret_cast<const uint2*>(s_head)[t];
        uint32_t m[4] = { hv.x & 0xffffu, hv.x >> 16, hv.y & 0xffffu, hv.y >> 16 };
        m[1] = max(m[0], m[1]); m[2] = max(m[1], m[2]); m[3] = max(m[2], m[3]);
        uint32_t scan = m[3];
#pragma unroll
        for (int o = 1; o < 64; o <<= 1) { const uint32_t v = __shfl_up(scan, o); if (lane >= o) scan = max(scan, v); }
        uint32_t before = __shfl_up(scan, 1);
        if (lane == 0) before = 0;
        if (lane == 63) s_wmax[wave] = scan;
        __syncthreads();
        before = max(before, carry);
        for (int w = 0; w < wave; w++) before = max(before, s_wmax[w]);
        carry = max(max(carry, max(s_wmax[0], s_wmax[1])), max(s_wmax[2], s_wmax[3]));
        const uint32_t o0 = c0 + 4u * t;
        K kq[4];
        uint32_t vq[4];
#pragma unroll
        for (int e = 0; e < 4; e++) {
            const uint32_t o = o0 + e;
            const uint32_t own = max(before, m[e]);
            kq[e] = 0; vq[e] = 0;
            if (o >= out_begin && o < out_end) {
                const int g = (int)own - 1;
                const uint32_t first = (g == 0) ? out_begin : s_end[g - 1];
                const uint2 rc = s_rect[g];
                const int x0 = rc.x & 0xffff, y0 = rc.x >> 16, x1 = rc.y & 0xffff;
                const uint32_t local = o - first, w = (uint32_t)(x1 - x0), inv = s_inv[g];
                const uint32_t ry = inv ? __umulhi(local, inv) : local, rx = local - ry * w;
                kq[e] = (K)((y0 + ry) * grid_x + (x0 + rx));
                vq[e] = s_id[g];
            }
        }
        if (o0 >= out_begin && o0 + 4 <= out_end) {
            if constexpr (sizeof(K) == 2)
                *reinterpret_cast<uint2*>(keys + o0) = make_uint2((uint32_t)kq[0] | ((uint32_t)kq[1] << 16), (uint32_t)kq[2] | ((uint32_t)kq[3] << 16));
            else
                *reinterpret_cast<uint4*>(keys + o0) = make_uint4((uint32_t)kq[0], (uint32_t)kq[1], (uint32_t)kq[2], (uint32_t)kq[3]);
            *reinterpret_cast<uint4*>(values + o0) = make_uint4(vq[0], vq[1], vq[2], vq[3]);
        } else {
#pragma unroll
            for (int e = 0; e < 4; e++)
                if (o0 + e >= out_begin && o0 + e < out_end) { keys[o0 + e] = kq[e]; values[o0 + e] = vq[e]; }
        }
        __syncthreads();
    }
}

void launch_depth_order_scan(int P, const GeomPtrs& g, hipStream_t s)
{
    if (P <= 0) return;
    const int nb = (P + 255) / 256;
    block_totals_kernel<<<nb, 256, 0, s>>>(P, g.sorted_offsets, g.depth_base);
    scan_blocks_kernel<<<1, 1024, 0, s>>>(nb, g.depth_base, nullptr, nullptr, 0u);
}

void launch_duplicate_with_keys(int P, const GeomPtrs& g, const BinPtrs& b, int grid_x, const uint32_t* sort_err,
                                void* zero_span, size_t zero_n16, hipStream_t s)
{
    if (P <= 0) return;
    if (!zero_span) zero_n16 = 0;
    if (b.key_bytes == 4)
        duplicate_with_keys_kernel<uint32_t><<<(P + 255) / 256, 256, 0, s>>>(P, g.depth_order, g.sorted_offsets, g.depth_base,
                                                                             (uint32_t*)b.keys_unsorted, b.values_unsorted, grid_x, sort_err, (uint4*)zero_span, zero_n16);
    else
        duplicate_with_keys_kernel<uint16_t><<<(P + 255) / 256, 256, 0, s>>>(P, g.depth_order, g.sorted_offsets, g.depth_base,
                                                                             (uint16_t*)b.keys_unsorted, b.values_unsorted, grid_x, sort_err, (uint4*)zero_span, zero_n16);
}

template <class K>
__global__ void __launch_bounds__(256)
identify_ranges_kernel(int L, const K* __restrict__ keys, uint2* __restrict__ ranges, const uint32_t* __restrict__ sort_err)
{
    if (*sort_err) return;
    const int j = blockIdx.x * 256 + threadIdx.x;
    const int i0 = j * 8;
    if (i0 >= L) return;
    uint32_t cur8[8];
    if constexpr (sizeof(K) == 2) {
        const uint4 v = reinterpret_cast<const uint4*>(keys)[j];
        const uint32_t w[4] = { v.x, v.y, v.z, v.w };
#pragma unroll
        for (int e = 0; e < 8; e++) cur8[e] = (e & 1) ? (w[e >> 1] >> 16) : (w[e >> 1] & 0xffffu);
    } else {
        const uint4 v0 = reinterpret_cast<const uint4*>(keys)[2 * j], v1 = reinterpret_cast<const uint4*>(keys)[2 * j + 1];
        cur8[0] = v0.x; cur8[1] = v0.y; cur8[2] = v0.z; cur8[3] = v0.w; cur8[4] = v1.x; cur8[5] = v1.y; cur8[6] = v1.z; cur8[7] = v1.w;
    }
    uint32_t prev = i0 > 0 ? (uint32_t)keys[i0 - 1] : 0xffffffffu;
#pragma unroll
    for (int e = 0; e < 8; e++) {
        const int idx = i0 + e;
        if (idx < L) {
            const uint32_t cur = cur8[e];
            if (cur != prev) {
                if (idx > 0) ranges[prev].y = (uint32_t)idx;
                ranges[cur].x = (uint32_t)idx;
            }
            if (idx == L - 1) ranges[cur].y = (uint32_t)L;
            prev = cur;
        }
    }
}

void launch_identify_ranges(int R, const void* keys_sorted, int key_bytes, uint2* ranges, const uint32_t* sort_err, hipStream_t s)
{
    if (R <= 0) return;
    const int threads = (R + 7) / 8;
    if (key_bytes == 4) identify_ranges_kernel<uint32_t><<<(threads + 255) / 256, 256, 0, s>>>(R, (const uint32_t*)keys_sorted, ranges, sort_err);
    else identify_ranges_kernel<uint16_t><<<(threads + 255) / 256, 256, 0, s>>>(R, (const uint16_t*)keys_sorted, ranges, sort_err);
}

}
```

c3dgs_amd/csrc/radix_sort.hip:

```cpp
#include "common.hpp"
#include <algorithm>
#include <cstdlib>

namespace c3dgs {

constexpr int OS_RADIX = 256;
#ifndef C3DGS_OS_TILE32
#define C3DGS_OS_TILE32 12288
#endif
#ifndef C3DGS_OS_BLOCK32
#define C3DGS_OS_BLOCK32 512
#endif
constexpr int OS_TILE16 = 8192, OS_BLOCK16 = 1024;
template <class K> struct OsShape {
    static constexpr int TILE = sizeof(K) == 2 ? OS_TILE16 : C3DGS_OS_TILE32;
    static constexpr int BLOCK = sizeof(K) == 2 ? OS_BLOCK16 : C3DGS_OS_BLOCK32;
    static constexpr int IPT = TILE / BLOCK;
};
constexpr uint32_t OS_FLAG_AGG = 1u << 30, OS_FLAG_PRE = 2u << 30, OS_CNT_MASK = (1u << 30) - 1;
constexpr int OS_MAX_PASSES = 4;
#ifndef C3DGS_OS_SPIN_LIMIT
#define C3DGS_OS_SPIN_LIMIT (1u << 22)
#endif
constexpr uint32_t OS_SPIN_LIMIT = C3DGS_OS_SPIN_LIMIT;
__device__ uint32_t g_os_error;
#ifdef C3DGS_OS_TIMING
__device__ unsigned long long g_os_times[64 * 8];
#define OS_T(slot) if (tid == 0 && (bid & 3) == 0 && (bid >> 2) < 64) g_os_times[(bid >> 2) * 8 + (slot)] = __builtin_readcyclecounter();
#else
#define OS_T(slot)
#endif

struct OsPlan { int passes; int bits[OS_MAX_PASSES]; };

static OsPlan os_plan(int total_bits)
{
    OsPlan p;
    p.passes = (total_bits + 7) / 8;
    if (p.passes < 1) p.passes = 1;
    int left = total_bits < 1 ? 1 : total_bits;
    for (int i = 0; i < p.passes; i++) {
        const int b = (left + (p.passes - i) - 1) / (p.passes - i);
        p.bits[i] = b;
        left -= b;
    }
    return p;
}

template <class K> static size_t os_blocks(size_t n) { return (n + OsShape<K>::TILE - 1) / OsShape<K>::TILE; }
template <class K> constexpr bool os_pre_pass0() { return sizeof(K) == 2; }
constexpr int OS_TABLE_ROW = 2 * OS_RADIX;
template <class K> static size_t os_table_words(size_t n) { return os_pre_pass0<K>() ? os_blocks<K>(n) * OS_TABLE_ROW : 0; }
template <class K> static size_t os_ctrl_bytes(size_t n, int passes)
{
    return align_up(((size_t)passes * OS_RADIX + (size_t)passes * os_blocks<K>(n) * OS_RADIX + 64 + os_table_words<K>(n)) * sizeof(uint32_t));
}

constexpr int OS_HIST_BLOCK = 1024;
template <class K>
__global__ void __launch_bounds__(OS_HIST_BLOCK) os_hist_kernel(const K* __restrict__ keys, size_t n, OsPlan plan, uint32_t* __restrict__ hist)
{
    __shared__ uint32_t s_h[OS_MAX_PASSES][OS_RADIX];
    for (int q = threadIdx.x; q < OS_MAX_PASSES * OS_RADIX; q += OS_HIST_BLOCK) (&s_h[0][0])[q] = 0;
    __syncthreads();
    constexpr int VEC = 16 / sizeof(K);
    const size_t nvec = n / VEC;
    const uint4* k4 = reinterpret_cast<const uint4*>(keys);
    auto add = [&](uint32_t k) {
        int shift = 0;
        for (int p = 0; p < plan.passes; p++) {
            atomicAdd(&s_h[p][(k >> shift) & ((1u << plan.bits[p]) - 1u)], 1u);
            shift += plan.bits[p];
        }
    };
    auto add4 = [&](const uint4 v) {
        const uint32_t w[4] = { v.x, v.y, v.z, v.w };
#pragma unroll
        for (int e = 0; e < 4; e++) {
            if (sizeof(K) == 4) add(w[e]);
            else { add(w[e] & 0xffffu); add(w[e] >> 16); }
        }
    };
    const size_t stride = (size_t)gridDim.x * OS_HIST_BLOCK;
    size_t i = (size_t)blockIdx.x * OS_HIST_BLOCK + threadIdx.x;
    for (; i + 3 * stride < nvec; i += 4 * stride) {
        const uint4 v0 = k4[i], v1 = k4[i + stride], v2 = k4[i + 2 * stride], v3 = k4[i + 3 * stride];
        add4(v0); add4(v1); add4(v2); add4(v3);
    }
    for (; i < nvec; i += stride) add4(k4[i]);
    for (size_t j = nvec * VEC + (size_t)blockIdx.x * OS_HIST_BLOCK + threadIdx.x; j < n; j += stride) add((uint32_t)keys[j]);
    __syncthreads();
    for (int q = threadIdx.x; q < plan.passes * OS_RADIX; q += OS_HIST_BLOCK) {
        const uint32_t v = (&s_h[0][0])[q];
        if (v) atomicAdd(&hist[q], v);
    }
}

__global__ void __launch_bounds__(1024) os_tile_hist_kernel(const uint16_t* __restrict__ keys, uint32_t n, OsPlan plan, uint32_t* __restrict__ table)
{
    constexpr int TILE = OsShape<uint16_t>::TILE;
    static_assert(TILE == 8 * 1024, "one 16-byte load of 8 keys per thread");
    __shared__ uint32_t s_h[OS_TABLE_ROW];
    if (threadIdx.x < OS_TABLE_ROW) s_h[threadIdx.x] = 0;
    __syncthreads();
    const uint32_t base = blockIdx.x * (uint32_t)TILE + threadIdx.x * 8u;
    const uint32_t m0 = (1u << plan.bits[0]) - 1u, m1 = plan.passes > 1 ? (1u << plan.bits[1]) - 1u : 0u;
    auto add = [&](uint32_t k) {
        atomicAdd(&s_h[k & m0], 1u);
        if (plan.passes > 1) atomicAdd(&s_h[OS_RADIX + ((k >> plan.bits[0]) & m1)], 1u);
    };
    if (base + 8 <= n && (reinterpret_cast<uintptr_t>(keys) & 15u) == 0) {
        const uint4 v = *reinterpret_cast<const uint4*>(keys + base);
        const uint32_t w[4] = { v.x, v.y, v.z, v.w };
#pragma unroll
        for (int e = 0; e < 4; e++) { add(w[e] & 0xffffu); add(w[e] >> 16); }
    } else {
        for (uint32_t i = base; i < min(base + 8u, n); i++) add((uint32_t)keys[i]);
    }
    __syncthreads();
    const int t = threadIdx.x;
    if (t < OS_TABLE_ROW && (t >> 8) < plan.passes && (t & (OS_RADIX - 1)) < (1 << plan.bits[(t >> 8) & 1]))
        table[(size_t)t * gridDim.x + blockIdx.x] = s_h[t];
}

__global__ void __launch_bounds__(256) os_table_scan_kernel(uint32_t* __restrict__ table, uint32_t blocks, OsPlan plan, uint32_t* __restrict__ hist)
{
    __shared__ uint32_t s_w[4];
    const int n0 = 1 << plan.bits[0];
    const int pass = (int)blockIdx.x < n0 ? 0 : 1, digit = (int)blockIdx.x - (pass ? n0 : 0), col = pass * OS_RADIX + digit;
    uint32_t* column = table + (size_t)col * blocks;
    const int lane = threadIdx.x & 63, wave = threadIdx.x >> 6;
    uint32_t carry = 0;
    for (uint32_t b0 = 0; b0 < blocks; b0 += 256) {
        const uint32_t b = b0 + threadIdx.x;
        const uint32_t c = b < blocks ? column[b] : 0u;
        uint32_t incl = c;
#pragma unroll
        for (int o = 1; o < 64; o <<= 1) { const uint32_t t = __shfl_up(incl, o); if (lane >= o) incl += t; }
        __syncthreads();
        if (lane == 63) s_w[wave] = incl;
        __syncthreads();
        uint32_t off = carry;
        for (int w = 0; w < wave; w++) off += s_w[w];
        if (pass == 0 && b < blocks) column[b] = off + incl - c;
        carry += s_w[0] + s_w[1] + s_w[2] + s_w[3];
    }
    if (threadIdx.x == 0) hist[col] = carry;
}

__device__ __forceinline__ uint32_t os_load(const uint32_t* p) { return __hip_atomic_load(p, __ATOMIC_RELAXED, __HIP_MEMORY_SCOPE_AGENT); }
__device__ __forceinline__ void os_store(uint32_t* p, uint32_t v) { __hip_atomic_store(p, v, __ATOMIC_RELAXED, __HIP_MEMORY_SCOPE_AGENT); }

__device__ __forceinline__ uint32_t os_pack_rect(uint2 r)
{
    return (r.x & 0xffu) | ((r.x >> 16) << 8) | ((r.y & 0xffu) << 16) | ((r.y >> 16) << 24);
}
__device__ __forceinline__ uint2 os_unpack_rect(uint32_t w)
{
    return make_uint2((w & 0xffu) | (((w >> 8) & 0xffu) << 16), ((w >> 16) & 0xffu) | ((w >> 24) << 16));
}

template <class K, int BITS, bool PRE, bool PAY2 = false>
__global__ void __launch_bounds__(OsShape<K>::BLOCK)
os_pass_kernel(const K* __restrict__ kin, K* __restrict__ kout, const uint32_t* __restrict__ vin, uint32_t* __restrict__ vout,
               uint32_t n, int shift, const uint32_t* __restrict__ hist, uint32_t* __restrict__ status, uint32_t* __restrict__ ticket,
               const uint2* __restrict__ gather_src, uint2* __restrict__ gather_dst, const uint32_t* __restrict__ p2in = nullptr,
               uint32_t* __restrict__ p2out = nullptr)
{
    constexpr uint32_t ERR_BIT = sizeof(K) == 2 ? 1u : 2u;
    constexpr uint32_t MASK = (1u << BITS) - 1;
    constexpr int OS_BLOCK = OsShape<K>::BLOCK, OS_IPT = OsShape<K>::IPT, OS_WAVES = OS_BLOCK / 64;
    __shared__ uint32_t s_cnt[OS_WAVES][OS_RADIX];
    __shared__ uint32_t s_start[OS_RADIX];
    __shared__ int32_t s_gbase[OS_RADIX];
    __shared__ uint32_t s_wtot[4];
    __shared__ uint32_t s_bid;
    constexpr int OS_TILE = OsShape<K>::TILE;
    __shared__ K s_keys[OS_TILE];
    __shared__ uint32_t s_vals[OS_TILE];
    __shared__ uint32_t s_vals2[PAY2 ? OS_TILE : 1];

    const int tid = threadIdx.x, lane = tid & 63, wave = tid >> 6;
    if (tid == 0) s_bid = PRE ? blockIdx.x : atomicAdd(ticket, 1u);
    for (int q = tid; q < OS_WAVES * OS_RADIX; q += OS_BLOCK) (&s_cnt[0][0])[q] = 0;
    __syncthreads();
    const uint32_t bid = s_bid;
    OS_T(0)
    const uint32_t block_start = bid * (uint32_t)OS_TILE;
    const uint32_t valid = min((uint32_t)OS_TILE, n - block_start);

    K key[OS_IPT];
    uint32_t val[OS_IPT], rank[OS_IPT];
    uint32_t val2[PAY2 ? OS_IPT : 1];
    const uint32_t wbase = block_start + (uint32_t)wave * 64u * OS_IPT;
#pragma unroll
    for (int k = 0; k < OS_IPT; k++) {
        const uint32_t idx = wbase + (uint32_t)k * 64u + lane;
        const bool ok = idx < n;
        key[k] = ok ? kin[idx] : (K)0;
        val[k] = ok ? (vin ? vin[idx] : idx) : 0u;
        if (PAY2) val2[k] = ok ? (p2in ? p2in[idx] : os_pack_rect(gather_src[idx])) : 0u;
    }
    const uint32_t lt_lo = lane < 32 ? (1u << lane) - 1u : 0xffffffffu, lt_hi = lane < 32 ? 0u : (1u << (lane - 32)) - 1u;
#ifdef C3DGS_OS_TIMING
    if (key[0] == (K)0x12345678 && val[OS_IPT - 1] == 0x87654321u) kout[0] = key[OS_IPT - 1];
    asm volatile("s_waitcnt vmcnt(0)");
#endif
    OS_T(1)
    uint32_t* wc = s_cnt[wave];
#pragma unroll
    for (int k = 0; k < OS_IPT; k++) {
        const uint32_t idx = wbase + (uint32_t)k * 64u + lane;
        const bool ok = idx < n;
        const uint32_t d = ((uint32_t)key[k] >> shift) & MASK;
        const unsigned long long okb = __ballot(ok);
        uint32_t plo = (uint32_t)okb, phi = (uint32_t)(okb >> 32);
#pragma unroll
        for (int b = 0; b < BITS; b++) {
            const int sgn = __builtin_amdgcn_sbfe((int)d, b, 1);
            const unsigned long long bal = __ballot(sgn != 0);
            plo &= ~((uint32_t)bal ^ (uint32_t)sgn);
            phi &= ~((uint32_t)(bal >> 32) ^ (uint32_t)sgn);
        }
        rank[k] = 0;
        if (ok) {
            const uint32_t before = __hip_atomic_load(&wc[d], __ATOMIC_RELAXED, __HIP_MEMORY_SCOPE_WAVEFRONT);
            const uint32_t below = (uint32_t)__popc(plo & lt_lo) + (uint32_t)__popc(phi & lt_hi);
            rank[k] = before + below;
            if (below == 0) __hip_atomic_store(&wc[d], before + (uint32_t)__popc(plo) + (uint32_t)__popc(phi), __ATOMIC_RELAXED, __HIP_MEMORY_SCOPE_WAVEFRONT);
        }
        __builtin_amdgcn_fence(__ATOMIC_RELEASE, "wavefront");
        __builtin_amdgcn_wave_barrier();
        __builtin_amdgcn_fence(__ATOMIC_ACQUIRE, "wavefront");
    }
    OS_T(2)
    __syncthreads();
    OS_T(3)
    uint32_t tot = 0;
    if (tid < OS_RADIX) {
#pragma unroll
        for (int w = 0; w < OS_WAVES; w++) { const uint32_t c = s_cnt[w][tid]; s_cnt[w][tid] = tot; tot += c; }
    }
    uint32_t incl = tot;
#pragma unroll
    for (int o = 1; o < 64; o <<= 1) { const uint32_t t = __shfl_up(incl, o); if (lane >= o) incl += t; }
    if (tid < OS_RADIX && lane == 63) s_wtot[wave] = incl;
    __syncthreads();
    uint32_t start = 0, pre = 0;
    if (tid < OS_RADIX) {
        uint32_t off = 0;
        for (int w = 0; w < wave; w++) off += s_wtot[w];
        start = off + incl - tot;
        s_start[tid] = start;
        uint32_t* my = status + (size_t)bid * OS_RADIX + tid;
        if (PRE) pre = tid < (1 << BITS) ? status[(size_t)tid * gridDim.x + bid] : 0u;
        else if (bid == 0) os_store(my, OS_FLAG_PRE | tot);
        else {
            os_store(my, OS_FLAG_AGG | tot);
            for (int64_t b = (int64_t)bid - 1;; b--) {
                uint32_t s, spins = 0;
                do { s = os_load(status + (size_t)b * OS_RADIX + tid); } while ((s >> 30) == 0 && ++spins < OS_SPIN_LIMIT);
                if ((s >> 30) == 0) { atomicOr(&g_os_error, ERR_BIT); break; }
                pre += s & OS_CNT_MASK;
                if (s & OS_FLAG_PRE) break;
            }
            os_store(my, OS_FLAG_PRE | (pre + tot));
        }
    }
    OS_T(4)
    const uint32_t h = tid < OS_RADIX ? hist[tid] : 0u;
    uint32_t hincl = h;
#pragma unroll
    for (int o = 1; o < 64; o <<= 1) { const uint32_t t = __shfl_up(hincl, o); if (lane >= o) hincl += t; }
    __syncthreads();
    if (tid < OS_RADIX && lane == 63) s_wtot[wave] = hincl;
    __syncthreads();
    if (tid < OS_RADIX) {
        uint32_t off = 0;
        for (int w = 0; w < wave; w++) off += s_wtot[w];
        s_gbase[tid] = (int32_t)(off + hincl - h + pre) - (int32_t)start;
    }
    OS_T(5)
#pragma unroll
    for (int k = 0; k < OS_IPT; k++) {
        const uint32_t idx = wbase + (uint32_t)k * 64u + lane;
        if (idx < n) {
            const uint32_t d = ((uint32_t)key[k] >> shift) & MASK;
            const uint32_t p = s_start[d] + s_cnt[wave][d] + rank[k];
            s_keys[p] = key[k];
            s_vals[p] = val[k];
            if (PAY2) s_vals2[p] = val2[k];
        }
    }
    __syncthreads();
    OS_T(6)
#pragma unroll
    for (int m = 0; m < OS_IPT; m++) {
        const uint32_t p = (uint32_t)tid + (uint32_t)m * OS_BLOCK;
        if (p < valid) {
            const K kk = s_keys[p];
            const uint32_t d = ((uint32_t)kk >> shift) & MASK;
            const uint32_t g = (uint32_t)(s_gbase[d] + (int32_t)p);
            kout[g] = kk;
            const uint32_t vv = s_vals[p];
            vout[g] = vv;
            if (PAY2) {
                if (p2out) p2out[g] = s_vals2[p];
                else gather_dst[g] = os_unpack_rect(s_vals2[p]);
            } else if (gather_src) gather_dst[g] = gather_src[vv];
        }
    }
#ifdef C3DGS_OS_TIMING
    asm volatile("s_waitcnt vmcnt(0)");
#endif
    OS_T(7)
}

template <class K, bool PRE>
static void os_launch_pass(int bits, unsigned blocks, hipStream_t s, const K* ki, K* ko, const uint32_t* vi, uint32_t* vo, uint32_t n,
                           int shift, const uint32_t* hist, uint32_t* status, uint32_t* ticket, const uint2* gsrc, uint2* gdst)
{
#define C3DGS_OS_CASE(B) case B: os_pass_kernel<K, B, PRE><<<blocks, OsShape<K>::BLOCK, 0, s>>>(ki, ko, vi, vo, n, shift, hist, status, ticket, gsrc, gdst); break
    switch (bits) {
        C3DGS_OS_CASE(1); C3DGS_OS_CASE(2); C3DGS_OS_CASE(3); C3DGS_OS_CASE(4);
        C3DGS_OS_CASE(5); C3DGS_OS_CASE(6); C3DGS_OS_CASE(7);
        default: os_pass_kernel<K, 8, PRE><<<blocks, OsShape<K>::BLOCK, 0, s>>>(ki, ko, vi, vo, n, shift, hist, status, ticket, gsrc, gdst); break;
    }
#undef C3DGS_OS_CASE
}

template <class K>
static size_t os_temp_bytes(size_t n, int total_bits, bool pay2 = false)
{
    const OsPlan plan = os_plan(total_bits);
    size_t b = os_ctrl_bytes<K>(n, plan.passes);
    const int bufs = plan.passes >= 3 ? 2 : (plan.passes == 2 ? 1 : 0);
    b += (size_t)bufs * (align_up(n * sizeof(K)) + align_up(n * sizeof(uint32_t)));
    if (pay2) b += 2 * align_up(n * sizeof(uint32_t));
    return b;
}

template <class K>
static size_t os_clear_bytes(size_t n, int total_bits)
{
    const OsPlan plan = os_plan(total_bits);
    if (!os_pre_pass0<K>()) return os_ctrl_bytes<K>(n, plan.passes);
    return ((size_t)plan.passes * OS_RADIX + (size_t)plan.passes * os_blocks<K>(n) * OS_RADIX + 64) * sizeof(uint32_t);
}

template <class K>
static hipError_t os_sort(void* temp, size_t temp_bytes, const K* kin, K* kout, const uint32_t* vin, uint32_t* vout, size_t n,
                          int total_bits, hipStream_t s, const uint2* gather_src = nullptr, uint2* gather_dst = nullptr,
                          bool ctrl_cleared = false, bool pay2 = false)
{
    if (n == 0) return hipSuccess;
    if (pay2 && (sizeof(K) != 4 || total_bits != 32 || !gather_src || !gather_dst || vin || os_temp_bytes<K>(n, total_bits, true) > temp_bytes))
        pay2 = false;
    if (n >= ((size_t)1 << 30) || os_temp_bytes<K>(n, total_bits) > temp_bytes) return hipErrorInvalidValue;
    const OsPlan plan = os_plan(total_bits);
    const size_t blocks = os_blocks<K>(n);
    char* base = (char*)temp;
    const size_t ctrl = os_ctrl_bytes<K>(n, plan.passes);
    uint32_t* hist = (uint32_t*)base;
    uint32_t* status = hist + (size_t)plan.passes * OS_RADIX;
    uint32_t* ticket = status + (size_t)plan.passes * blocks * OS_RADIX;
    uint32_t* table = ticket + 64;
    constexpr bool pre0 = os_pre_pass0<K>();
    K* tk[2]; uint32_t* tv[2];
    char* q = base + ctrl;
    for (int i = 0; i < 2; i++) { tk[i] = (K*)q; q += align_up(n * sizeof(K)); tv[i] = (uint32_t*)q; q += align_up(n * sizeof(uint32_t)); }
    uint32_t* t2[2] = { nullptr, nullptr };
    if (pay2) {
        q = base + os_temp_bytes<K>(n, total_bits);
        for (int i = 0; i < 2; i++) { t2[i] = (uint32_t*)q; q += align_up(n * sizeof(uint32_t)); }
    }
    if (!ctrl_cleared) {
        const hipError_t e = hipMemsetAsync(base, 0, os_clear_bytes<K>(n, total_bits), s);
        if (e != hipSuccess) return e;
    }
    if constexpr (pre0) {
        os_tile_hist_kernel<<<(unsigned)blocks, 1024, 0, s>>>((const uint16_t*)kin, (uint32_t)n, plan, table);
        os_table_scan_kernel<<<(unsigned)((1 << plan.bits[0]) + (plan.passes > 1 ? (1 << plan.bits[1]) : 0)), 256, 0, s>>>(table, (uint32_t)blocks, plan, hist);
    } else {
        const size_t nvec16 = n * sizeof(K) / 16 + 1;
        const unsigned hb = (unsigned)std::min<size_t>((nvec16 + OS_HIST_BLOCK * 4 - 1) / (OS_HIST_BLOCK * 4), 512);
        os_hist_kernel<K><<<hb, OS_HIST_BLOCK, 0, s>>>(kin, n, plan, hist);
    }
    int shift = 0;
    for (int p = 0; p < plan.passes; p++) {
        const K* ki = p == 0 ? kin : tk[(p - 1) & 1];
        const uint32_t* vi = p == 0 ? vin : tv[(p - 1) & 1];
        K* ko = p == plan.passes - 1 ? kout : tk[p & 1];
        uint32_t* vo = p == plan.passes - 1 ? vout : tv[p & 1];
        const bool last = p == plan.passes - 1;
        if constexpr (sizeof(K) == 4) {
            if (pay2) {
                os_pass_kernel<K, 8, false, true><<<(unsigned)blocks, OsShape<K>::BLOCK, 0, s>>>(
                    ki, ko, vi, vo, (uint32_t)n, shift, hist + (size_t)p * OS_RADIX, status + (size_t)p * blocks * OS_RADIX, ticket + p,
                    gather_src, gather_dst, p == 0 ? nullptr : t2[(p - 1) & 1], last ? nullptr : t2[p & 1]);
                shift += plan.bits[p];
                continue;
            }
        }
        if (pre0 && p == 0)
            os_launch_pass<K, true>(plan.bits[p], (unsigned)blocks, s, ki, ko, vi, vo, (uint32_t)n, shift, hist, table, ticket,
                                    last ? gather_src : nullptr, last ? gather_dst : nullptr);
        else
            os_launch_pass<K, false>(plan.bits[p], (unsigned)blocks, s, ki, ko, vi, vo, (uint32_t)n, shift, hist + (size_t)p * OS_RADIX,
                                     status + (size_t)p * blocks * OS_RADIX, ticket + p, last ? gather_src : nullptr, last ? gather_dst : nullptr);
        shift += plan.bits[p];
    }
    return hipGetLastError();
}

#ifdef C3DGS_OS_TIMING
int os_read_times(unsigned long long* out512)
{
    return hipMemcpyFromSymbol(out512, HIP_SYMBOL(g_os_times), sizeof(unsigned long long) * 512) != hipSuccess;
}
#else
int os_read_times(unsigned long long*) { return 1; }
#endif

uint32_t* onesweep_error_word()
{
    static uint32_t* cache[64] = { nullptr };
    int dev = 0;
    if (hipGetDevice(&dev) != hipSuccess || dev < 0 || dev >= 64) return nullptr;
    if (!cache[dev]) {
        void* p = nullptr;
        if (hipGetSymbolAddress(&p, HIP_SYMBOL(g_os_error)) != hipSuccess) return nullptr;
        cache[dev] = (uint32_t*)p;
    }
    return cache[dev];
}

int onesweep_timed_out(hipStream_t s)
{
    if (!onesweep_enabled()) return 0;
    uint32_t* e = onesweep_error_word();
    uint32_t w = 1;
    if (!e || hipMemcpyAsync(&w, e, sizeof(w), hipMemcpyDeviceToHost, s) != hipSuccess) return 1;
    if (hipStreamSynchronize(s) != hipSuccess) return 1;
    if (w) (void)hipMemsetAsync(e, 0, sizeof(w), s);
    return w != 0;
}

bool onesweep_enabled()
{
    static const bool on = []() { const char* e = std::getenv("C3DGS_SORT_ROCPRIM"); return !(e && e[0] == '1'); }();
    return on;
}
size_t onesweep_depth_temp_bytes(int P) { return os_temp_bytes<uint32_t>((size_t)(P > 0 ? P : 1), 32, true); }
size_t onesweep_tile_temp_bytes(int R, int end_bit, int key_bytes)
{
    return key_bytes == 4 ? os_temp_bytes<uint32_t>((size_t)(R > 0 ? R : 1), end_bit) : os_temp_bytes<uint16_t>((size_t)(R > 0 ? R : 1), end_bit);
}
size_t onesweep_depth_clear_bytes(int P) { return os_clear_bytes<uint32_t>((size_t)(P > 0 ? P : 1), 32); }
size_t onesweep_tile_clear_bytes(int R, int end_bit, int key_bytes)
{
    return key_bytes == 4 ? os_clear_bytes<uint32_t>((size_t)(R > 0 ? R : 1), end_bit) : os_clear_bytes<uint16_t>((size_t)(R > 0 ? R : 1), end_bit);
}
hipError_t onesweep_tile_sort32(void* temp, size_t temp_bytes, const uint32_t* kin, uint32_t* kout, const uint32_t* vin, uint32_t* vout,
                                int R, int end_bit, hipStream_t s, bool ctrl_cleared)
{
    return os_sort<uint32_t>(temp, temp_bytes, kin, kout, vin, vout, (size_t)R, end_bit, s, nullptr, nullptr, ctrl_cleared);
}
hipError_t onesweep_depth_sort(void* temp, size_t temp_bytes, const uint32_t* kin, uint32_t* kout, const uint32_t* vin, uint32_t* vout,
                               int P, const uint2* gather_src, uint2* gather_dst, hipStream_t s, bool ctrl_cleared, bool rects_fit_bytes)
{
    static const bool no_pay2 = []() { const char* e = std::getenv("C3DGS_DEPTH_SORT_GATHER"); return e && e[0] == '1'; }();
    return os_sort<uint32_t>(temp, temp_bytes, kin, kout, vin, vout, (size_t)P, 32, s, gather_src, gather_dst, ctrl_cleared,
                             rects_fit_bytes && !no_pay2);
}
hipError_t onesweep_tile_sort(void* temp, size_t temp_bytes, const uint16_t* kin, uint16_t* kout, const uint32_t* vin, uint32_t* vout,
                              int R, int end_bit, hipStream_t s, bool ctrl_cleared)
{
    return os_sort<uint16_t>(temp, temp_bytes, kin, kout, vin, vout, (size_t)R, end_bit, s, nullptr, nullptr, ctrl_cleared);
}

}
```

Baseline: 592.5 views/s.

## Range-compress depth sort keys and use adaptive 9-bit onesweep passes

```diff
diff --git a/c3dgs_amd/csrc/binning.hip b/c3dgs_amd/csrc/binning.hip
--- a/c3dgs_amd/csrc/binning.hip
+++ b/c3dgs_amd/csrc/binning.hip
@@ -47,12 +47,18 @@
     return (onesweep_enabled() && (size_t)R < ((size_t)1 << 30)) ? onesweep_tile_clear_bytes(R, end_bit, key_bytes) : 0;
 }
 
+uint2* depth_sort_key_ranges(void* temp, int P)
+{
+    return (onesweep_enabled() && (size_t)P < ((size_t)1 << 30)) ? onesweep_depth_ranges(temp, P) : nullptr;
+}
+
 hipError_t run_depth_sort(void* temp, size_t temp_bytes, const uint32_t* kin, uint32_t* kout, const uint32_t* vin,
                           uint32_t* vout, int P, const uint2* rects, uint2* rects_sorted, hipStream_t s, bool ctrl_cleared,
-                          bool rects_fit_bytes)
+                          bool rects_fit_bytes, bool ranges_ready)
 {
     if (onesweep_enabled() && (size_t)P < ((size_t)1 << 30))
-        return onesweep_depth_sort(temp, temp_bytes, kin, kout, vin, vout, P, rects, rects_sorted, s, ctrl_cleared, rects_fit_bytes);
+        return onesweep_depth_sort(temp, temp_bytes, kin, kout, vin, vout, P, rects, rects_sorted, s, ctrl_cleared, rects_fit_bytes,
+                                   ranges_ready);
     hipError_t e = vin ? rocprim::radix_sort_pairs(temp, temp_bytes, kin, kout, vin, vout, (size_t)P, 0u, 32u, s)
                        : rocprim::radix_sort_pairs(temp, temp_bytes, kin, kout, rocprim::counting_iterator<uint32_t>(0u), vout,
                                                    (size_t)P, 0u, 32u, s);
diff --git a/c3dgs_amd/csrc/c_abi.hip b/c3dgs_amd/csrc/c_abi.hip
--- a/c3dgs_amd/csrc/c_abi.hip
+++ b/c3dgs_amd/csrc/c_abi.hip
@@ -143,9 +143,10 @@
     if (hr.dev && seq == 0u) hr.seq = 1u;
     const uint32_t want_seq = hr.dev ? hr.seq : 0u;
     const size_t dclear = depth_sort_clear_bytes(P) <= g.scan_temp_bytes ? depth_sort_clear_bytes(P) : 0;
+    uint2* key_ranges = depth_sort_key_ranges(g.scan_temp, P);
     { StageTimer t_(ST_PREPROCESS, s);
       if (geom_gtab_bytes(p)) launch_pack_codebook(p, g.gtab, s);
-      launch_preprocess(p, g, radii, img.ranges, sort_err, g.scan_temp, dclear / 16, hr.dev, want_seq, s); }
+      launch_preprocess(p, g, radii, img.ranges, sort_err, g.scan_temp, dclear / 16, hr.dev, want_seq, key_ranges, s); }
     C3DGS_STAGE("preprocess", p.debug, s);
     if (!hr.dev) {
         C3DGS_HIP_TRY(hipMemcpyAsync(hr.pinned, g.block_base + (P + 255) / 256, 2 * sizeof(uint32_t), hipMemcpyDeviceToHost, s));
@@ -154,7 +155,7 @@
     { StageTimer t_(ST_DEPTH_SORT, s);
       C3DGS_HIP_TRY(run_depth_sort(g.scan_temp, g.scan_temp_bytes, g.depth_keys, g.depth_keys_sorted, nullptr, g.depth_order, P,
                                    reinterpret_cast<const uint2*>(g.rects), g.sorted_offsets, s, dclear != 0,
-                                   gx <= 255 && gy <= 255)); }
+                                   gx <= 255 && gy <= 255, key_ranges != nullptr)); }
     C3DGS_STAGE("depth_sort", p.debug, s);
     if (p.debug && onesweep_timed_out(s)) return fail(C3DGS_E_HIP, "depth sort: look-back timed out");
     { StageTimer t_(ST_SCAN, s); launch_depth_order_scan(P, g, s); }
diff --git a/c3dgs_amd/csrc/common.hpp b/c3dgs_amd/csrc/common.hpp
--- a/c3dgs_amd/csrc/common.hpp
+++ b/c3dgs_amd/csrc/common.hpp
@@ -140,14 +140,15 @@
 void launch_mark_visible_pose(int P, const float* means3D, const float* pose7, uint8_t* present, hipStream_t s);
 void launch_pack_codebook(const c3dgs_raster_params& p, float4* gtab, hipStream_t s);
 void launch_preprocess(const c3dgs_raster_params& p, const GeomPtrs& g, int32_t* radii, uint2* ranges, const uint32_t* sort_err,
-                       void* zero_span, size_t zero_n16, uint32_t* host_out, uint32_t host_seq, hipStream_t s);
+                       void* zero_span, size_t zero_n16, uint32_t* host_out, uint32_t host_seq, uint2* key_ranges, hipStream_t s);
 void launch_depth_order_scan(int P, const GeomPtrs& g, hipStream_t s);
 void launch_duplicate_with_keys(int P, const GeomPtrs& g, const BinPtrs& b, int grid_x, const uint32_t* sort_err,
                                 void* zero_span, size_t zero_n16, hipStream_t s);
 void launch_identify_ranges(int R, const void* keys_sorted, int key_bytes, uint2* ranges, const uint32_t* sort_err, hipStream_t s);
 hipError_t run_depth_sort(void* temp, size_t temp_bytes, const uint32_t* kin, uint32_t* kout, const uint32_t* vin,
                           uint32_t* vout, int P, const uint2* rects, uint2* rects_sorted, hipStream_t s, bool ctrl_cleared = false,
-                          bool rects_fit_bytes = false);
+                          bool rects_fit_bytes = false, bool ranges_ready = false);
+uint2* depth_sort_key_ranges(void* temp, int P);
 hipError_t run_tile_sort(void* temp, size_t temp_bytes, const void* kin, void* kout, int key_bytes, const uint32_t* vin,
                          uint32_t* vout, int R, int end_bit, hipStream_t s, bool ctrl_cleared = false);
 size_t depth_sort_clear_bytes(int P);
@@ -158,10 +159,11 @@
 size_t onesweep_depth_temp_bytes(int P);
 size_t onesweep_tile_temp_bytes(int R, int end_bit, int key_bytes = 2);
 size_t onesweep_depth_clear_bytes(int P);
+uint2* onesweep_depth_ranges(void* temp, int P);
 size_t onesweep_tile_clear_bytes(int R, int end_bit, int key_bytes);
 hipError_t onesweep_depth_sort(void* temp, size_t temp_bytes, const uint32_t* kin, uint32_t* kout, const uint32_t* vin, uint32_t* vout,
                                int P, const uint2* gather_src, uint2* gather_dst, hipStream_t s, bool ctrl_cleared = false,
-                               bool rects_fit_bytes = false);
+                               bool rects_fit_bytes = false, bool ranges_ready = false);
 hipError_t onesweep_tile_sort32(void* temp, size_t temp_bytes, const uint32_t* kin, uint32_t* kout, const uint32_t* vin, uint32_t* vout,
                                 int R, int end_bit, hipStream_t s, bool ctrl_cleared = false);
 hipError_t onesweep_tile_sort(void* temp, size_t temp_bytes, const uint16_t* kin, uint16_t* kout, const uint32_t* vin, uint32_t* vout,
diff --git a/c3dgs_amd/csrc/preprocess.hip b/c3dgs_amd/csrc/preprocess.hip
--- a/c3dgs_amd/csrc/preprocess.hip
+++ b/c3dgs_amd/csrc/preprocess.hip
@@ -142,12 +142,13 @@
     uint2* ranges; int T;
     const float4* gtab;
     uint4* zero_span; size_t zero_n16;
+    uint2* key_range;
 };
 
 template <int DEG>
 __global__ void __launch_bounds__(256) preprocess_kernel(const PreArgs a)
 {
-    __shared__ uint32_t s_wsum[4];
+    __shared__ uint32_t s_wsum[4], s_klo[4], s_khi[4];
     const int t = threadIdx.x, lane = t & 63, wave = t >> 6;
     const int i = blockIdx.x * 256 + t;
     const bool in_range = i < a.P;
@@ -254,11 +255,20 @@
 #pragma unroll
     for (int o = 1; o < 64; o <<= 1) { const uint32_t v = __shfl_up(incl, o); if (lane >= o) incl += v; }
     if (lane == 63) s_wsum[wave] = incl;
+    uint32_t klo = out_key, khi = out_key == 0xffffffffu ? 0u : out_key;
+    if (a.key_range) {
+#pragma unroll
+        for (int o = 32; o > 0; o >>= 1) { klo = min(klo, (uint32_t)__shfl_xor((int)klo, o)); khi = max(khi, (uint32_t)__shfl_xor((int)khi, o)); }
+        if (lane == 0) { s_klo[wave] = klo; s_khi[wave] = khi; }
+    }
     __syncthreads();
     uint32_t woff = 0;
     for (int w = 0; w < wave; w++) woff += s_wsum[w];
     const uint32_t my_incl = woff + incl;
     if (t == 255) a.block_total[blockIdx.x] = my_incl;
+    if (t == 0 && a.key_range)
+        a.key_range[blockIdx.x] = make_uint2(min(min(s_klo[0], s_klo[1]), min(s_klo[2], s_klo[3])),
+                                             max(max(s_khi[0], s_khi[1]), max(s_khi[2], s_khi[3])));
     if (!in_range) return;
     if (!alive) *reinterpret_cast<uint2*>(a.rects + 4 * (size_t)i) = make_uint2(0u, 0u);
     if (alive) {
@@ -273,10 +283,11 @@
 }
 
 __global__ void __launch_bounds__(1024) scan_blocks_kernel(int nb, uint32_t* __restrict__ base, const uint32_t* __restrict__ sort_err,
-                                                           uint32_t* __restrict__ host_out, uint32_t host_seq)
-{
-    __shared__ uint32_t s_w[2][16];
+                                                           uint32_t* __restrict__ host_out, uint32_t host_seq, uint2* __restrict__ key_range)
+{
+    __shared__ uint32_t s_w[2][16], s_klo[16], s_khi[16];
     const int t = threadIdx.x, lane = t & 63, wave = t >> 6;
+    uint32_t klo = 0xffffffffu, khi = 0u;
     uint32_t carry = 0;
     int buf = 0;
     for (int c0 = 0; c0 < nb; c0 += 16384, buf ^= 1) {
@@ -293,6 +304,19 @@
             }
             v[4 * q] = x.x; v[4 * q + 1] = x.y; v[4 * q + 2] = x.z; v[4 * q + 3] = x.w;
         }
+        if (key_range) {
+#pragma unroll
+            for (int q = 0; q < 8; q++) {
+                const int j = i0 + 2 * q;
+                if (j + 1 < nb) {
+                    const uint4 x = reinterpret_cast<const uint4*>(key_range + i0)[q];
+                    klo = min(klo, min(x.x, x.z)); khi = max(khi, max(x.y, x.w));
+                } else if (j < nb) {
+                    const uint2 x = key_range[j];
+                    klo = min(klo, x.x); khi = max(khi, x.y);
+                }
+            }
+        }
         uint32_t mine = 0;
 #pragma unroll
         for (int q = 0; q < 16; q++) mine += v[q];
@@ -318,7 +342,16 @@
         }
         carry += all;
     }
+    if (key_range) {
+#pragma unroll
+        for (int o = 32; o > 0; o >>= 1) { klo = min(klo, (uint32_t)__shfl_xor((int)klo, o)); khi = max(khi, (uint32_t)__shfl_xor((int)khi, o)); }
+        if (lane == 0) { s_klo[wave] = klo; s_khi[wave] = khi; }
+    }
     __syncthreads();
+    if (t == 0 && key_range) {
+        for (int w = 1; w < 16; w++) { klo = min(klo, s_klo[w]); khi = max(khi, s_khi[w]); }
+        key_range[nb] = make_uint2(klo, khi);
+    }
     if (t == 0) {
         base[nb] = carry;
         const uint32_t err = sort_err ? *sort_err : 0u;
@@ -332,7 +365,7 @@
 }
 
 void launch_preprocess(const c3dgs_raster_params& p, const GeomPtrs& g, int32_t* radii, uint2* ranges, const uint32_t* sort_err,
-                       void* zero_span, size_t zero_n16, uint32_t* host_out, uint32_t host_seq, hipStream_t s)
+                       void* zero_span, size_t zero_n16, uint32_t* host_out, uint32_t host_seq, uint2* key_ranges, hipStream_t s)
 {
     if (p.P <= 0) return;
     PreArgs a;
@@ -352,6 +385,7 @@
     a.ranges = ranges; a.T = a.gx * a.gy;
     a.gtab = g.gtab;
     a.zero_span = (uint4*)zero_span; a.zero_n16 = zero_span ? zero_n16 : 0;
+    a.key_range = key_ranges;
     const dim3 grid((p.P + 255) / 256), block(256);
     const int deg = p.colors_precomp ? 0 : p.D;
     switch (deg) {
@@ -360,7 +394,7 @@
         case 2: preprocess_kernel<2><<<grid, block, 0, s>>>(a); break;
         default: preprocess_kernel<3><<<grid, block, 0, s>>>(a); break;
     }
-    scan_blocks_kernel<<<1, 1024, 0, s>>>((int)grid.x, g.block_base, sort_err, host_out, host_seq);
+    scan_blocks_kernel<<<1, 1024, 0, s>>>((int)grid.x, g.block_base, sort_err, host_out, host_seq, key_ranges);
 }
 
 __device__ __forceinline__ uint32_t rect_tiles(const uint2 rc)
@@ -482,7 +516,7 @@
     if (P <= 0) return;
     const int nb = (P + 255) / 256;
     block_totals_kernel<<<nb, 256, 0, s>>>(P, g.sorted_offsets, g.depth_base);
-    scan_blocks_kernel<<<1, 1024, 0, s>>>(nb, g.depth_base, nullptr, nullptr, 0u);
+    scan_blocks_kernel<<<1, 1024, 0, s>>>(nb, g.depth_base, nullptr, nullptr, 0u, nullptr);
 }
 
 void launch_duplicate_with_keys(int P, const GeomPtrs& g, const BinPtrs& b, int grid_x, const uint32_t* sort_err,
diff --git a/c3dgs_amd/csrc/radix_sort.hip b/c3dgs_amd/csrc/radix_sort.hip
--- a/c3dgs_amd/csrc/radix_sort.hip
+++ b/c3dgs_amd/csrc/radix_sort.hip
@@ -6,7 +6,7 @@
 
 constexpr int OS_RADIX = 256;
 #ifndef C3DGS_OS_TILE32
-#define C3DGS_OS_TILE32 12288
+#define C3DGS_OS_TILE32 11776
 #endif
 #ifndef C3DGS_OS_BLOCK32
 #define C3DGS_OS_BLOCK32 512
@@ -17,6 +17,14 @@
     static constexpr int BLOCK = sizeof(K) == 2 ? OS_BLOCK16 : C3DGS_OS_BLOCK32;
     static constexpr int IPT = TILE / BLOCK;
 };
+template <class K> constexpr size_t os_pass_lds(int radix, bool pay2)
+{
+    return (size_t)(OsShape<K>::BLOCK / 64) * radix * 4 + 2 * (size_t)radix * 4 + (size_t)(radix / 64) * 4 + 4 +
+           (size_t)OsShape<K>::TILE * (sizeof(K) + 4 + (pay2 ? 4 : 0)) + (pay2 ? 0 : 4);
+}
+static_assert(OsShape<uint32_t>::TILE % OsShape<uint32_t>::BLOCK == 0, "whole items per thread");
+static_assert(os_pass_lds<uint32_t>(512, true) <= 160 * 1024, "depth pass (9-bit digits, second payload) exceeds the LDS of a CU");
+static_assert(os_pass_lds<uint16_t>(256, false) <= 160 * 1024, "tile pass exceeds the LDS of a CU");
 constexpr uint32_t OS_FLAG_AGG = 1u << 30, OS_FLAG_PRE = 2u << 30, OS_CNT_MASK = (1u << 30) - 1;
 constexpr int OS_MAX_PASSES = 4;
 #ifndef C3DGS_OS_SPIN_LIMIT
@@ -47,6 +55,30 @@
     return p;
 }
 
+constexpr int OS_DRADIX = 512;
+constexpr int OS_RANGE_GROUP = 256;
+struct OsDepthPlan { uint32_t passes, lo, culled, pad; uint32_t bits[OS_MAX_PASSES]; uint32_t shift[OS_MAX_PASSES]; };
+__host__ __device__ inline OsDepthPlan os_depth_plan(uint32_t lo, uint32_t hi)
+{
+    OsDepthPlan q = {};
+    const uint32_t span = lo <= hi ? hi - lo + 1u : 0u;
+    q.lo = lo <= hi ? lo : 0u;
+    q.culled = span;
+    int b = 0;
+    for (uint32_t v = span; v; v >>= 1) b++;
+    if (b < 1) b = 1;
+    q.passes = b <= 27 ? (uint32_t)((b + 8) / 9) : 4u;
+    int left = b, shift = 0;
+    for (int i = 0; i < (int)q.passes; i++) {
+        const int w = (left + ((int)q.passes - i) - 1) / ((int)q.passes - i);
+        q.bits[i] = (uint32_t)w; q.shift[i] = (uint32_t)shift;
+        left -= w; shift += w;
+    }
+    return q;
+}
+__device__ __forceinline__ uint32_t os_depth_rank_key(uint32_t k, uint32_t lo, uint32_t culled) { return k == 0xffffffffu ? culled : k - lo; }
+static size_t os_depth_ranges(size_t n) { return (n + OS_RANGE_GROUP - 1) / OS_RANGE_GROUP; }
+
 template <class K> static size_t os_blocks(size_t n) { return (n + OsShape<K>::TILE - 1) / OsShape<K>::TILE; }
 template <class K> constexpr bool os_pre_pass0() { return sizeof(K) == 2; }
 constexpr int OS_TABLE_ROW = 2 * OS_RADIX;
@@ -148,6 +180,60 @@
     if (threadIdx.x == 0) hist[col] = carry;
 }
 
+__global__ void __launch_bounds__(OS_RANGE_GROUP) os_range_kernel(const uint32_t* __restrict__ keys, uint32_t n, uint2* __restrict__ ranges)
+{
+    __shared__ uint32_t s_lo[OS_RANGE_GROUP / 64], s_hi[OS_RANGE_GROUP / 64];
+    const uint32_t i = blockIdx.x * OS_RANGE_GROUP + threadIdx.x;
+    const uint32_t k = i < n ? keys[i] : 0xffffffffu;
+    uint32_t lo = k, hi = k == 0xffffffffu ? 0u : k;
+#pragma unroll
+    for (int o = 32; o > 0; o >>= 1) { lo = min(lo, (uint32_t)__shfl_xor((int)lo, o)); hi = max(hi, (uint32_t)__shfl_xor((int)hi, o)); }
+    if ((threadIdx.x & 63) == 0) { s_lo[threadIdx.x >> 6] = lo; s_hi[threadIdx.x >> 6] = hi; }
+    __syncthreads();
+    if (threadIdx.x == 0) {
+        for (int w = 1; w < OS_RANGE_GROUP / 64; w++) { lo = min(lo, s_lo[w]); hi = max(hi, s_hi[w]); }
+        ranges[blockIdx.x] = make_uint2(lo, hi);
+    }
+}
+
+__global__ void __launch_bounds__(OS_HIST_BLOCK) os_depth_hist_kernel(const uint32_t* __restrict__ keys, uint32_t n, const uint2* __restrict__ ranges,
+                                                                      uint32_t nranges, OsDepthPlan* __restrict__ plan_out, uint32_t* __restrict__ hist)
+{
+    __shared__ uint32_t s_h[OS_MAX_PASSES][OS_DRADIX];
+    __shared__ uint32_t s_lo[OS_HIST_BLOCK / 64], s_hi[OS_HIST_BLOCK / 64];
+    for (int q = threadIdx.x; q < OS_MAX_PASSES * OS_DRADIX; q += OS_HIST_BLOCK) (&s_h[0][0])[q] = 0;
+    uint32_t lo = 0xffffffffu, hi = 0u;
+    for (uint32_t r = threadIdx.x; r < nranges; r += OS_HIST_BLOCK) { const uint2 v = ranges[r]; lo = min(lo, v.x); hi = max(hi, v.y); }
+#pragma unroll
+    for (int o = 32; o > 0; o >>= 1) { lo = min(lo, (uint32_t)__shfl_xor((int)lo, o)); hi = max(hi, (uint32_t)__shfl_xor((int)hi, o)); }
+    if ((threadIdx.x & 63) == 0) { s_lo[threadIdx.x >> 6] = lo; s_hi[threadIdx.x >> 6] = hi; }
+    __syncthreads();
+    for (int w = 0; w < OS_HIST_BLOCK / 64; w++) { lo = min(lo, s_lo[w]); hi = max(hi, s_hi[w]); }
+    const OsDepthPlan plan = os_depth_plan(lo, hi);
+    if (blockIdx.x == 0 && threadIdx.x == 0) *plan_out = plan;
+    const int passes = (int)plan.passes;
+    auto add = [&](uint32_t k) {
+        const uint32_t x = os_depth_rank_key(k, plan.lo, plan.culled);
+        for (int p = 0; p < passes; p++) atomicAdd(&s_h[p][(x >> plan.shift[p]) & ((1u << plan.bits[p]) - 1u)], 1u);
+    };
+    auto add4 = [&](const uint4 v) { add(v.x); add(v.y); add(v.z); add(v.w); };
+    const uint32_t nvec = n / 4;
+    const uint4* k4 = reinterpret_cast<const uint4*>(keys);
+    const uint32_t stride = gridDim.x * OS_HIST_BLOCK;
+    uint32_t i = blockIdx.x * OS_HIST_BLOCK + threadIdx.x;
+    for (; i + 3 * stride < nvec; i += 4 * stride) {
+        const uint4 v0 = k4[i], v1 = k4[i + stride], v2 = k4[i + 2 * stride], v3 = k4[i + 3 * stride];
+        add4(v0); add4(v1); add4(v2); add4(v3);
+    }
+    for (; i < nvec; i += stride) add4(k4[i]);
+    for (uint32_t j = nvec * 4 + blockIdx.x * OS_HIST_BLOCK + threadIdx.x; j < n; j += stride) add(keys[j]);
+    __syncthreads();
+    for (int q = threadIdx.x; q < passes * OS_DRADIX; q += OS_HIST_BLOCK) {
+        const uint32_t v = (&s_h[0][0])[q];
+        if (v) atomicAdd(&hist[q], v);
+    }
+}
+
 __device__ __forceinline__ uint32_t os_load(const uint32_t* p) { return __hip_atomic_load(p, __ATOMIC_RELAXED, __HIP_MEMORY_SCOPE_AGENT); }
 __device__ __forceinline__ void os_store(uint32_t* p, uint32_t v) { __hip_atomic_store(p, v, __ATOMIC_RELAXED, __HIP_MEMORY_SCOPE_AGENT); }
 
@@ -160,20 +246,41 @@
     return make_uint2((w & 0xffu) | (((w >> 8) & 0xffu) << 16), ((w >> 16) & 0xffu) | ((w >> 24) << 16));
 }
 
-template <class K, int BITS, bool PRE, bool PAY2 = false>
+template <class K, int BITS, bool PRE, bool PAY2 = false, bool DEV = false>
 __global__ void __launch_bounds__(OsShape<K>::BLOCK)
 os_pass_kernel(const K* __restrict__ kin, K* __restrict__ kout, const uint32_t* __restrict__ vin, uint32_t* __restrict__ vout,
                uint32_t n, int shift, const uint32_t* __restrict__ hist, uint32_t* __restrict__ status, uint32_t* __restrict__ ticket,
                const uint2* __restrict__ gather_src, uint2* __restrict__ gather_dst, const uint32_t* __restrict__ p2in = nullptr,
-               uint32_t* __restrict__ p2out = nullptr)
+               uint32_t* __restrict__ p2out = nullptr, const OsDepthPlan* __restrict__ dplan = nullptr, int pass = 0,
+               K* __restrict__ kfin = nullptr, uint32_t* __restrict__ vfin = nullptr)
 {
     constexpr uint32_t ERR_BIT = sizeof(K) == 2 ? 1u : 2u;
-    constexpr uint32_t MASK = (1u << BITS) - 1;
+    constexpr int RADIX = DEV ? OS_DRADIX : OS_RADIX;
+    static_assert(!DEV || (sizeof(K) == 4 && BITS == 9 && !PRE && OsShape<K>::BLOCK >= OS_DRADIX), "depth pass shape");
+    static_assert(DEV || BITS <= 8, "8-bit digits outside the depth sort");
     constexpr int OS_BLOCK = OsShape<K>::BLOCK, OS_IPT = OsShape<K>::IPT, OS_WAVES = OS_BLOCK / 64;
-    __shared__ uint32_t s_cnt[OS_WAVES][OS_RADIX];
-    __shared__ uint32_t s_start[OS_RADIX];
-    __shared__ int32_t s_gbase[OS_RADIX];
-    __shared__ uint32_t s_wtot[4];
+    int nbits = BITS;
+    uint32_t lo = 0, culled = 0;
+    if constexpr (DEV) {
+        const uint32_t passes = dplan->passes;
+        if ((uint32_t)pass >= passes) return;
+        nbits = (int)dplan->bits[pass];
+        shift = (int)dplan->shift[pass];
+        lo = dplan->lo; culled = dplan->culled;
+        if ((uint32_t)pass == passes - 1) { kout = kfin; vout = vfin; p2out = nullptr; }
+        else if (!PAY2) gather_src = nullptr;
+    }
+    const uint32_t MASK = (1u << nbits) - 1u;
+    const int ndig = 1 << nbits;
+    auto digit = [&](K k) -> uint32_t {
+        uint32_t x = (uint32_t)k;
+        if constexpr (DEV) x = os_depth_rank_key(x, lo, culled);
+        return (x >> shift) & MASK;
+    };
+    __shared__ uint32_t s_cnt[OS_WAVES][RADIX];
+    __shared__ uint32_t s_start[RADIX];
+    __shared__ int32_t s_gbase[RADIX];
+    __shared__ uint32_t s_wtot[RADIX / 64];
     __shared__ uint32_t s_bid;
     constexpr int OS_TILE = OsShape<K>::TILE;
     __shared__ K s_keys[OS_TILE];
@@ -182,7 +289,7 @@
 
     const int tid = threadIdx.x, lane = tid & 63, wave = tid >> 6;
     if (tid == 0) s_bid = PRE ? blockIdx.x : atomicAdd(ticket, 1u);
-    for (int q = tid; q < OS_WAVES * OS_RADIX; q += OS_BLOCK) (&s_cnt[0][0])[q] = 0;
+    for (int q = tid; q < OS_WAVES * RADIX; q += OS_BLOCK) (&s_cnt[0][0])[q] = 0;
     __syncthreads();
     const uint32_t bid = s_bid;
     OS_T(0)
@@ -212,15 +319,17 @@
     for (int k = 0; k < OS_IPT; k++) {
         const uint32_t idx = wbase + (uint32_t)k * 64u + lane;
         const bool ok = idx < n;
-        const uint32_t d = ((uint32_t)key[k] >> shift) & MASK;
+        const uint32_t d = digit(key[k]);
         const unsigned long long okb = __ballot(ok);
         uint32_t plo = (uint32_t)okb, phi = (uint32_t)(okb >> 32);
 #pragma unroll
         for (int b = 0; b < BITS; b++) {
-            const int sgn = __builtin_amdgcn_sbfe((int)d, b, 1);
-            const unsigned long long bal = __ballot(sgn != 0);
-            plo &= ~((uint32_t)bal ^ (uint32_t)sgn);
-            phi &= ~((uint32_t)(bal >> 32) ^ (uint32_t)sgn);
+            if (!DEV || b < nbits) {
+                const int sgn = __builtin_amdgcn_sbfe((int)d, b, 1);
+                const unsigned long long bal = __ballot(sgn != 0);
+                plo &= ~((uint32_t)bal ^ (uint32_t)sgn);
+                phi &= ~((uint32_t)(bal >> 32) ^ (uint32_t)sgn);
+            }
         }
         rank[k] = 0;
         if (ok) {
@@ -237,29 +346,30 @@
     __syncthreads();
     OS_T(3)
     uint32_t tot = 0;
-    if (tid < OS_RADIX) {
+    if (tid < RADIX) {
 #pragma unroll
         for (int w = 0; w < OS_WAVES; w++) { const uint32_t c = s_cnt[w][tid]; s_cnt[w][tid] = tot; tot += c; }
     }
     uint32_t incl = tot;
 #pragma unroll
     for (int o = 1; o < 64; o <<= 1) { const uint32_t t = __shfl_up(incl, o); if (lane >= o) incl += t; }
-    if (tid < OS_RADIX && lane == 63) s_wtot[wave] = incl;
+    if (tid < RADIX && lane == 63) s_wtot[wave] = incl;
     __syncthreads();
     uint32_t start = 0, pre = 0;
-    if (tid < OS_RADIX) {
+    if (tid < RADIX) {
         uint32_t off = 0;
         for (int w = 0; w < wave; w++) off += s_wtot[w];
         start = off + incl - tot;
         s_start[tid] = start;
-        uint32_t* my = status + (size_t)bid * OS_RADIX + tid;
+        uint32_t* my = status + (size_t)bid * RADIX + tid;
         if (PRE) pre = tid < (1 << BITS) ? status[(size_t)tid * gridDim.x + bid] : 0u;
+        else if (DEV && tid >= ndig) { }
         else if (bid == 0) os_store(my, OS_FLAG_PRE | tot);
         else {
             os_store(my, OS_FLAG_AGG | tot);
             for (int64_t b = (int64_t)bid - 1;; b--) {
                 uint32_t s, spins = 0;
-                do { s = os_load(status + (size_t)b * OS_RADIX + tid); } while ((s >> 30) == 0 && ++spins < OS_SPIN_LIMIT);
+                do { s = os_load(status + (size_t)b * RADIX + tid); } while ((s >> 30) == 0 && ++spins < OS_SPIN_LIMIT);
                 if ((s >> 30) == 0) { atomicOr(&g_os_error, ERR_BIT); break; }
                 pre += s & OS_CNT_MASK;
                 if (s & OS_FLAG_PRE) break;
@@ -268,14 +378,14 @@
         }
     }
     OS_T(4)
-    const uint32_t h = tid < OS_RADIX ? hist[tid] : 0u;
+    const uint32_t h = tid < RADIX ? hist[tid] : 0u;
     uint32_t hincl = h;
 #pragma unroll
     for (int o = 1; o < 64; o <<= 1) { const uint32_t t = __shfl_up(hincl, o); if (lane >= o) hincl += t; }
     __syncthreads();
-    if (tid < OS_RADIX && lane == 63) s_wtot[wave] = hincl;
-    __syncthreads();
-    if (tid < OS_RADIX) {
+    if (tid < RADIX && lane == 63) s_wtot[wave] = hincl;
+    __syncthreads();
+    if (tid < RADIX) {
         uint32_t off = 0;
         for (int w = 0; w < wave; w++) off += s_wtot[w];
         s_gbase[tid] = (int32_t)(off + hincl - h + pre) - (int32_t)start;
@@ -285,7 +395,7 @@
     for (int k = 0; k < OS_IPT; k++) {
         const uint32_t idx = wbase + (uint32_t)k * 64u + lane;
         if (idx < n) {
-            const uint32_t d = ((uint32_t)key[k] >> shift) & MASK;
+            const uint32_t d = digit(key[k]);
             const uint32_t p = s_start[d] + s_cnt[wave][d] + rank[k];
             s_keys[p] = key[k];
             s_vals[p] = val[k];
@@ -299,7 +409,7 @@
         const uint32_t p = (uint32_t)tid + (uint32_t)m * OS_BLOCK;
         if (p < valid) {
             const K kk = s_keys[p];
-            const uint32_t d = ((uint32_t)kk >> shift) & MASK;
+            const uint32_t d = digit(kk);
             const uint32_t g = (uint32_t)(s_gbase[d] + (int32_t)p);
             kout[g] = kk;
             const uint32_t vv = s_vals[p];
@@ -330,13 +440,12 @@
 }
 
 template <class K>
-static size_t os_temp_bytes(size_t n, int total_bits, bool pay2 = false)
+static size_t os_temp_bytes(size_t n, int total_bits)
 {
     const OsPlan plan = os_plan(total_bits);
     size_t b = os_ctrl_bytes<K>(n, plan.passes);
     const int bufs = plan.passes >= 3 ? 2 : (plan.passes == 2 ? 1 : 0);
     b += (size_t)bufs * (align_up(n * sizeof(K)) + align_up(n * sizeof(uint32_t)));
-    if (pay2) b += 2 * align_up(n * sizeof(uint32_t));
     return b;
 }
 
@@ -351,11 +460,9 @@
 template <class K>
 static hipError_t os_sort(void* temp, size_t temp_bytes, const K* kin, K* kout, const uint32_t* vin, uint32_t* vout, size_t n,
                           int total_bits, hipStream_t s, const uint2* gather_src = nullptr, uint2* gather_dst = nullptr,
-                          bool ctrl_cleared = false, bool pay2 = false)
+                          bool ctrl_cleared = false)
 {
     if (n == 0) return hipSuccess;
-    if (pay2 && (sizeof(K) != 4 || total_bits != 32 || !gather_src || !gather_dst || vin || os_temp_bytes<K>(n, total_bits, true) > temp_bytes))
-        pay2 = false;
     if (n >= ((size_t)1 << 30) || os_temp_bytes<K>(n, total_bits) > temp_bytes) return hipErrorInvalidValue;
     const OsPlan plan = os_plan(total_bits);
     const size_t blocks = os_blocks<K>(n);
@@ -369,11 +476,6 @@
     K* tk[2]; uint32_t* tv[2];
     char* q = base + ctrl;
     for (int i = 0; i < 2; i++) { tk[i] = (K*)q; q += align_up(n * sizeof(K)); tv[i] = (uint32_t*)q; q += align_up(n * sizeof(uint32_t)); }
-    uint32_t* t2[2] = { nullptr, nullptr };
-    if (pay2) {
-        q = base + os_temp_bytes<K>(n, total_bits);
-        for (int i = 0; i < 2; i++) { t2[i] = (uint32_t*)q; q += align_up(n * sizeof(uint32_t)); }
-    }
     if (!ctrl_cleared) {
         const hipError_t e = hipMemsetAsync(base, 0, os_clear_bytes<K>(n, total_bits), s);
         if (e != hipSuccess) return e;
@@ -393,15 +495,6 @@
         K* ko = p == plan.passes - 1 ? kout : tk[p & 1];
         uint32_t* vo = p == plan.passes - 1 ? vout : tv[p & 1];
         const bool last = p == plan.passes - 1;
-        if constexpr (sizeof(K) == 4) {
-            if (pay2) {
-                os_pass_kernel<K, 8, false, true><<<(unsigned)blocks, OsShape<K>::BLOCK, 0, s>>>(
-                    ki, ko, vi, vo, (uint32_t)n, shift, hist + (size_t)p * OS_RADIX, status + (size_t)p * blocks * OS_RADIX, ticket + p,
-                    gather_src, gather_dst, p == 0 ? nullptr : t2[(p - 1) & 1], last ? nullptr : t2[p & 1]);
-                shift += plan.bits[p];
-                continue;
-            }
-        }
         if (pre0 && p == 0)
             os_launch_pass<K, true>(plan.bits[p], (unsigned)blocks, s, ki, ko, vi, vo, (uint32_t)n, shift, hist, table, ticket,
                                     last ? gather_src : nullptr, last ? gather_dst : nullptr);
@@ -413,6 +506,54 @@
     return hipGetLastError();
 }
 
+static size_t os_depth_clear(size_t n) { return ((size_t)OS_MAX_PASSES * OS_DRADIX * (1 + os_blocks<uint32_t>(n)) + 64) * sizeof(uint32_t); }
+static size_t os_depth_plan_off(size_t n) { return align_up(os_depth_clear(n)); }
+static size_t os_depth_ranges_off(size_t n) { return os_depth_plan_off(n) + align_up(sizeof(OsDepthPlan)); }
+static size_t os_depth_ctrl(size_t n) { return align_up(os_depth_ranges_off(n) + (os_depth_ranges(n) + 1) * sizeof(uint2)); }
+static size_t os_depth_temp(size_t n, bool pay2) { return os_depth_ctrl(n) + (size_t)(pay2 ? 6 : 4) * align_up(n * sizeof(uint32_t)); }
+
+static hipError_t os_depth_sort(void* temp, size_t temp_bytes, const uint32_t* kin, uint32_t* kout, const uint32_t* vin, uint32_t* vout,
+                                size_t n, hipStream_t s, const uint2* gather_src, uint2* gather_dst, bool ctrl_cleared, bool pay2,
+                                bool ranges_ready)
+{
+    if (n == 0) return hipSuccess;
+    if (pay2 && (!gather_src || !gather_dst || vin || os_depth_temp(n, true) > temp_bytes)) pay2 = false;
+    if (n >= ((size_t)1 << 30) || os_depth_temp(n, false) > temp_bytes) return hipErrorInvalidValue;
+    const size_t blocks = os_blocks<uint32_t>(n), nranges = os_depth_ranges(n);
+    char* base = (char*)temp;
+    uint32_t* hist = (uint32_t*)base;
+    uint32_t* status = hist + (size_t)OS_MAX_PASSES * OS_DRADIX;
+    uint32_t* ticket = status + (size_t)OS_MAX_PASSES * blocks * OS_DRADIX;
+    OsDepthPlan* plan = (OsDepthPlan*)(base + os_depth_plan_off(n));
+    uint2* ranges = (uint2*)(base + os_depth_ranges_off(n));
+    uint32_t* tk[2]; uint32_t* tv[2]; uint32_t* t2[2] = { nullptr, nullptr };
+    char* q = base + os_depth_ctrl(n);
+    for (int i = 0; i < 2; i++) { tk[i] = (uint32_t*)q; q += align_up(n * 4); tv[i] = (uint32_t*)q; q += align_up(n * 4); }
+    if (pay2) for (int i = 0; i < 2; i++) { t2[i] = (uint32_t*)q; q += align_up(n * 4); }
+    if (!ctrl_cleared) {
+        const hipError_t e = hipMemsetAsync(base, 0, os_depth_clear(n), s);
+        if (e != hipSuccess) return e;
+    }
+    if (!ranges_ready) os_range_kernel<<<(unsigned)nranges, OS_RANGE_GROUP, 0, s>>>(kin, (uint32_t)n, ranges);
+    const unsigned hb = (unsigned)std::min<size_t>((n / 4 + 1 + OS_HIST_BLOCK * 4 - 1) / (OS_HIST_BLOCK * 4), 512);
+    os_depth_hist_kernel<<<hb, OS_HIST_BLOCK, 0, s>>>(kin, (uint32_t)n, ranges_ready ? ranges + nranges : ranges,
+                                                      ranges_ready ? 1u : (uint32_t)nranges, plan, hist);
+    for (int p = 0; p < OS_MAX_PASSES; p++) {
+        const uint32_t* ki = p == 0 ? kin : tk[(p - 1) & 1];
+        const uint32_t* vi = p == 0 ? vin : tv[(p - 1) & 1];
+        uint32_t* h = hist + (size_t)p * OS_DRADIX;
+        uint32_t* st = status + (size_t)p * blocks * OS_DRADIX;
+        if (pay2)
+            os_pass_kernel<uint32_t, 9, false, true, true><<<(unsigned)blocks, OsShape<uint32_t>::BLOCK, 0, s>>>(
+                ki, tk[p & 1], vi, tv[p & 1], (uint32_t)n, 0, h, st, ticket + p, gather_src, gather_dst,
+                p == 0 ? nullptr : t2[(p - 1) & 1], t2[p & 1], plan, p, kout, vout);
+        else
+            os_pass_kernel<uint32_t, 9, false, false, true><<<(unsigned)blocks, OsShape<uint32_t>::BLOCK, 0, s>>>(
+                ki, tk[p & 1], vi, tv[p & 1], (uint32_t)n, 0, h, st, ticket + p, gather_src, gather_dst, nullptr, nullptr, plan, p, kout, vout);
+    }
+    return hipGetLastError();
+}
+
 #ifdef C3DGS_OS_TIMING
 int os_read_times(unsigned long long* out512)
 {
@@ -451,12 +592,13 @@
     static const bool on = []() { const char* e = std::getenv("C3DGS_SORT_ROCPRIM"); return !(e && e[0] == '1'); }();
     return on;
 }
-size_t onesweep_depth_temp_bytes(int P) { return os_temp_bytes<uint32_t>((size_t)(P > 0 ? P : 1), 32, true); }
+size_t onesweep_depth_temp_bytes(int P) { return os_depth_temp((size_t)(P > 0 ? P : 1), true); }
+uint2* onesweep_depth_ranges(void* temp, int P) { return (uint2*)((char*)temp + os_depth_ranges_off((size_t)(P > 0 ? P : 1))); }
 size_t onesweep_tile_temp_bytes(int R, int end_bit, int key_bytes)
 {
     return key_bytes == 4 ? os_temp_bytes<uint32_t>((size_t)(R > 0 ? R : 1), end_bit) : os_temp_bytes<uint16_t>((size_t)(R > 0 ? R : 1), end_bit);
 }
-size_t onesweep_depth_clear_bytes(int P) { return os_clear_bytes<uint32_t>((size_t)(P > 0 ? P : 1), 32); }
+size_t onesweep_depth_clear_bytes(int P) { return os_depth_clear((size_t)(P > 0 ? P : 1)); }
 size_t onesweep_tile_clear_bytes(int R, int end_bit, int key_bytes)
 {
     return key_bytes == 4 ? os_clear_bytes<uint32_t>((size_t)(R > 0 ? R : 1), end_bit) : os_clear_bytes<uint16_t>((size_t)(R > 0 ? R : 1), end_bit);
@@ -467,11 +609,12 @@
     return os_sort<uint32_t>(temp, temp_bytes, kin, kout, vin, vout, (size_t)R, end_bit, s, nullptr, nullptr, ctrl_cleared);
 }
 hipError_t onesweep_depth_sort(void* temp, size_t temp_bytes, const uint32_t* kin, uint32_t* kout, const uint32_t* vin, uint32_t* vout,
-                               int P, const uint2* gather_src, uint2* gather_dst, hipStream_t s, bool ctrl_cleared, bool rects_fit_bytes)
+                               int P, const uint2* gather_src, uint2* gather_dst, hipStream_t s, bool ctrl_cleared, bool rects_fit_bytes,
+                               bool ranges_ready)
 {
     static const bool no_pay2 = []() { const char* e = std::getenv("C3DGS_DEPTH_SORT_GATHER"); return e && e[0] == '1'; }();
-    return os_sort<uint32_t>(temp, temp_bytes, kin, kout, vin, vout, (size_t)P, 32, s, gather_src, gather_dst, ctrl_cleared,
-                             rects_fit_bytes && !no_pay2);
+    return os_depth_sort(temp, temp_bytes, kin, kout, vin, vout, (size_t)P, s, gather_src, gather_dst, ctrl_cleared,
+                         rects_fit_bytes && !no_pay2, ranges_ready);
 }
 hipError_t onesweep_tile_sort(void* temp, size_t temp_bytes, const uint16_t* kin, uint16_t* kout, const uint32_t* vin, uint32_t* vout,
                               int R, int end_bit, hipStream_t s, bool ctrl_cleared)
```

Result: no change. 593.5 views/s (median of 4 runs) (+0.2%).
